# qcraftai/gedepth

Hardware: AMD Instinct MI355X
Metric: training img/s (whole node), KITTI-shaped 352x1120 synthetic batches (higher is better)
Workload: dtype bf16; 1 GPU; depthformer_swint_v: DepthFormer-SwinT + GEDepth-Vanilla, 352x1120, 8 img/GPU, full train step; global_batch=8, parallelism=dp1, allreduce_dtype=fp32, layout=nhwc, window_attention=bf16 mfma, params=53516992, hip_graph=off

## Files before the change

gedepth_amd/csrc/nhwc.hip:

```cpp
#include "common.h"

#define NH_MAXLANES 256

#define NH_MAXBLOCKS 1024
template <int K, int VN>
__device__ __forceinline__ void nh_col_commit(float (&acc)[K][VN], float* __restrict__ partial, int C, int lpr, int rpi, int c0) {
  __shared__ float sm[K][NH_MAXLANES][VN];
  const int t = threadIdx.x, rs = t / lpr;
#pragma unroll
  for (int k = 0; k < K; ++k)
#pragma unroll
    for (int v = 0; v < VN; ++v) sm[k][t][v] = acc[k][v];
  __syncthreads();
  int span = 1;
  while (span < rpi) span <<= 1;
  for (int stride = span >> 1; stride > 0; stride >>= 1) {
    if (rs < stride && rs + stride < rpi) {
#pragma unroll
      for (int k = 0; k < K; ++k)
#pragma unroll
        for (int v = 0; v < VN; ++v) sm[k][t][v] += sm[k][t + stride * lpr][v];
    }
    __syncthreads();
  }
  if (t < lpr) {
#pragma unroll
    for (int k = 0; k < K; ++k) {
      float* o = partial + ((long)blockIdx.x * K + k) * C + c0;
#pragma unroll
      for (int v = 0; v < VN; v += 4) *(float4*)(o + v) = make_float4(sm[k][t][v], sm[k][t][v + 1], sm[k][t][v + 2], sm[k][t][v + 3]);
    }
  }
}
template <typename O>
__global__ void __launch_bounds__(256) nh_partials_reduce_k(const float* __restrict__ partial, O* __restrict__ ws, int KC, int nb, int accumulate) {
  __shared__ double sm[8][32];
  const int j = threadIdx.x & 31, sl = threadIdx.x >> 5;
  const int kc = blockIdx.x * 32 + j;
  double a = 0.0;
  if (kc < KC) {
#pragma unroll 8
    for (int b = sl; b < nb; b += 8) a += (double)partial[(long)b * KC + kc];
  }
  sm[sl][j] = a;
  __syncthreads();
  if (sl == 0 && kc < KC) {
#pragma unroll
    for (int q = 1; q < 8; ++q) a += sm[q][j];
    ws[kc] = accumulate ? (O)((double)ws[kc] + a) : (O)a;
  }
}
static inline unsigned nh_grid_rows(long R, int rpi) { return ge_blocks(R, rpi * 8, NH_MAXBLOCKS); }
extern "C" size_t ge_nhwc_workspace(int C, int K) {
  return (size_t)C * ((size_t)K * sizeof(double) + 3 * sizeof(float) + (size_t)NH_MAXBLOCKS * K * sizeof(float));
}
static inline float* nh_partials(void* workspace, int C, int K) { return (float*)((char*)workspace + (size_t)C * (K * sizeof(double) + 3 * sizeof(float))); }
static inline void nh_reduce_launch_f32(void* workspace, int C, unsigned nb, float* out, int accumulate, hipStream_t s) {
  nh_partials_reduce_k<float><<<(C + 31) / 32, 256, 0, s>>>(nh_partials(workspace, C, 1), out, C, (int)nb, accumulate);
}
static inline void nh_reduce_launch(void* workspace, int C, int K, unsigned nb, hipStream_t s) {
  nh_partials_reduce_k<double><<<(K * C + 31) / 32, 256, 0, s>>>(nh_partials(workspace, C, K), (double*)workspace, K * C, (int)nb, 0);
}

template <typename T>
__global__ void __launch_bounds__(256) bn_stats_nhwc_k(const T* __restrict__ x, float* __restrict__ ws, int C, long R, int lpr, int rpi) {
  constexpr int VN = V8<T>::N;
  const int t = threadIdx.x, lane = t % lpr, rs = t / lpr;
  const int c0 = lane * VN;
  float acc[2][VN];
#pragma unroll
  for (int v = 0; v < VN; ++v) { acc[0][v] = 0.f; acc[1][v] = 0.f; }
  if (rs < rpi)
    for (long r = (long)blockIdx.x * rpi + rs; r < R; r += (long)gridDim.x * rpi) {
      float v[VN];
      V8<T>::ld(x + r * C + c0, v);
#pragma unroll
      for (int k = 0; k < VN; ++k) { acc[0][k] += v[k]; acc[1][k] += v[k] * v[k]; }
    }
  nh_col_commit<2, VN>(acc, ws, C, lpr, rpi, c0);
}
template <typename T>
__global__ void __launch_bounds__(256) bn_apply_nhwc_k(const T* __restrict__ x, const float* __restrict__ coef, T* __restrict__ y, int C,
                                                       long R, int lpr, int rpi, float slope) {
  constexpr int VN = V8<T>::N;
  const int t = threadIdx.x, lane = t % lpr, rs = t / lpr;
  if (rs >= rpi) return;
  const int c0 = lane * VN;
  float a[VN], b[VN];
#pragma unroll
  for (int k = 0; k < VN; ++k) { a[k] = coef[c0 + k]; b[k] = coef[C + c0 + k]; }
  for (long r = (long)blockIdx.x * rpi + rs; r < R; r += (long)gridDim.x * rpi) {
    float v[VN];
    V8<T>::ld(x + r * C + c0, v);
#pragma unroll
    for (int k = 0; k < VN; ++k) { const float tv = __fmaf_rn(v[k], a[k], b[k]); v[k] = tv > 0.f ? tv : tv * slope; }
    V8<T>::st(y + r * C + c0, v);
  }
}
template <typename T, bool RECOMP>
__global__ void __launch_bounds__(256) bn_bwd_stats_nhwc_k(const T* __restrict__ dy, const T* __restrict__ y, const T* __restrict__ x,
                                                           const float* __restrict__ gamma, const float* __restrict__ beta,
                                                           const float* __restrict__ save_mean, const float* __restrict__ save_rstd,
                                                           float* __restrict__ ws, int C, long R, int lpr, int rpi, float slope) {
  constexpr int VN = V8<T>::N;
  const int t = threadIdx.x, lane = t % lpr, rs = t / lpr;
  const int c0 = lane * VN;
  float mu[VN], rsd[VN], acc[2][VN], fa[VN], fb[VN];
#pragma unroll
  for (int v = 0; v < VN; ++v) {
    mu[v] = save_mean[c0 + v]; rsd[v] = save_rstd[c0 + v]; acc[0][v] = 0.f; acc[1][v] = 0.f;
    if (RECOMP) { fa[v] = gamma[c0 + v] * rsd[v]; fb[v] = __fmaf_rn(-mu[v], fa[v], beta[c0 + v]); }
  }
  if (rs < rpi)
    for (long r = (long)blockIdx.x * rpi + rs; r < R; r += (long)gridDim.x * rpi) {
      float g[VN], yv[VN], xv[VN];
      V8<T>::ld(dy + r * C + c0, g);
      V8<T>::ld(x + r * C + c0, xv);
      if (RECOMP) {
#pragma unroll
        for (int k = 0; k < VN; ++k) yv[k] = __fmaf_rn(xv[k], fa[k], fb[k]);
      } else {
        V8<T>::ld(y + r * C + c0, yv);
      }
#pragma unroll
      for (int k = 0; k < VN; ++k) {
        const float gg = yv[k] > 0.f ? g[k] : g[k] * slope;
        acc[0][k] += gg;
        acc[1][k] += gg * ((xv[k] - mu[k]) * rsd[k]);
      }
    }
  nh_col_commit<2, VN>(acc, ws, C, lpr, rpi, c0);
}
template <typename T, bool RECOMP>
__global__ void __launch_bounds__(256) bn_bwd_apply_nhwc_k(const T* __restrict__ dy, const T* __restrict__ y, const T* __restrict__ x,
                                                           const float* __restrict__ beta, const float* __restrict__ save_mean,
                                                           const float* __restrict__ save_rstd, const float* __restrict__ coef,
                                                           T* __restrict__ dx, int C, long R, int lpr, int rpi, float slope) {
  constexpr int VN = V8<T>::N;
  const int t = threadIdx.x, lane = t % lpr, rs = t / lpr;
  if (rs >= rpi) return;
  const int c0 = lane * VN;
  float a[VN], m1[VN], m2[VN], mu[VN], rsd[VN], fb[VN];
#pragma unroll
  for (int k = 0; k < VN; ++k) {
    a[k] = coef[c0 + k]; m1[k] = coef[C + c0 + k]; m2[k] = coef[2 * C + c0 + k]; mu[k] = save_mean[c0 + k]; rsd[k] = save_rstd[c0 + k];
    if (RECOMP) fb[k] = __fmaf_rn(-mu[k], a[k], beta[c0 + k]);
  }
  for (long r = (long)blockIdx.x * rpi + rs; r < R; r += (long)gridDim.x * rpi) {
    float g[VN], yv[VN], xv[VN];
    V8<T>::ld(dy + r * C + c0, g);
    V8<T>::ld(x + r * C + c0, xv);
    if (RECOMP) {
#pragma unroll
      for (int k = 0; k < VN; ++k) yv[k] = __fmaf_rn(xv[k], a[k], fb[k]);
    } else {
      V8<T>::ld(y + r * C + c0, yv);
    }
#pragma unroll
    for (int k = 0; k < VN; ++k) {
      const float gg = yv[k] > 0.f ? g[k] : g[k] * slope;
      g[k] = a[k] * (gg - m1[k] - ((xv[k] - mu[k]) * rsd[k]) * m2[k]);
    }
    V8<T>::st(dx + r * C + c0, g);
  }
}

__global__ void __launch_bounds__(256) bn_finalize_nhwc_k(const double* __restrict__ ws, const float* __restrict__ gamma,
                                                          const float* __restrict__ beta, float* __restrict__ save_mean,
                                                          float* __restrict__ save_rstd, float* __restrict__ running_mean,
                                                          float* __restrict__ running_var, float* __restrict__ coef, int C, double n,
                                                          float eps, float momentum) {
  const int c = blockIdx.x * blockDim.x + threadIdx.x;
  if (c >= C) return;
  const double mean = ws[c] / n;
  double var = ws[C + c] / n - mean * mean;
  if (var < 0.0) var = 0.0;
  const float rstd = (float)(1.0 / sqrt(var + (double)eps));
  save_mean[c] = (float)mean;
  save_rstd[c] = rstd;
  if (running_mean) running_mean[c] = (1.f - momentum) * running_mean[c] + momentum * (float)mean;
  if (running_var) running_var[c] = (1.f - momentum) * running_var[c] + momentum * (float)(n > 1.0 ? var * n / (n - 1.0) : var);
  const float a = gamma[c] * rstd;
  coef[c] = a;
  coef[C + c] = __fmaf_rn(-(float)mean, a, beta[c]);
}
__global__ void __launch_bounds__(256) bn_bwd_finalize_nhwc_k(const double* __restrict__ ws, const float* __restrict__ gamma,
                                                              const float* __restrict__ save_rstd, float* __restrict__ dgamma,
                                                              float* __restrict__ dbeta, float* __restrict__ coef, int C, double n) {
  const int c = blockIdx.x * blockDim.x + threadIdx.x;
  if (c >= C) return;
  dbeta[c] = (float)ws[c];
  dgamma[c] = (float)ws[C + c];
  coef[c] = gamma[c] * save_rstd[c];
  coef[C + c] = (float)(ws[c] / n);
  coef[2 * C + c] = (float)(ws[C + c] / n);
}

template <typename T> static bool nh_geom(int C, int& lpr, int& rpi) {
  constexpr int VN = V8<T>::N;
  if (C <= 0 || C % VN) return false;
  lpr = C / VN;
  if (lpr > NH_MAXLANES) return false;
  rpi = NH_MAXLANES / lpr;
  return true;
}
static inline bool nh_aligned(const void* a, const void* b = nullptr, const void* c = nullptr, const void* d = nullptr) {
  return ((((uintptr_t)a) | ((uintptr_t)b) | ((uintptr_t)c) | ((uintptr_t)d)) & 15) == 0;
}
static inline unsigned nh_grid_vec(long nvec) { return ge_blocks(nvec, 256 * 4, 65536); }
static inline unsigned nh_grid_apply(long R, int rpi) { return ge_blocks(R, rpi * 4, 16384); }

template <typename T>
static int bn_nhwc_fwd_launch(const void* x, const float* gamma, const float* beta, void* y, float* save_mean, float* save_rstd,
                              float* running_mean, float* running_var, void* workspace, long R, int C, float eps, float momentum,
                              float slope, hipStream_t s) {
  int lpr, rpi;
  if (!nh_geom<T>(C, lpr, rpi) || !nh_aligned(x, y)) return GE_ERR_UNSUPPORTED;
  double* ws = (double*)workspace;
  float* coef = (float*)(ws + 2 * C);
  const unsigned nb = nh_grid_rows(R, rpi);
  bn_stats_nhwc_k<T><<<nb, 256, 0, s>>>((const T*)x, nh_partials(workspace, C, 2), C, R, lpr, rpi);
  GE_LAUNCH_CHECK();
  nh_reduce_launch(workspace, C, 2, nb, s);
  GE_LAUNCH_CHECK();
  bn_finalize_nhwc_k<<<(C + 255) / 256, 256, 0, s>>>(ws, gamma, beta, save_mean, save_rstd, running_mean, running_var, coef, C, (double)R, eps, momentum);
  GE_LAUNCH_CHECK();
  bn_apply_nhwc_k<T><<<nh_grid_apply(R, rpi), 256, 0, s>>>((const T*)x, coef, (T*)y, C, R, lpr, rpi, slope);
  GE_LAUNCH_CHECK();
  return GE_OK;
}
template <typename T>
static int bn_nhwc_bwd_launch(const void* dy, const void* y, const void* x, const float* gamma, const float* beta, const float* save_mean,
                              const float* save_rstd, void* dx, float* dgamma, float* dbeta, void* workspace, long R, int C, float slope,
                              hipStream_t s) {
  int lpr, rpi;
  if (!nh_geom<T>(C, lpr, rpi) || !nh_aligned(dy, y, x, dx)) return GE_ERR_UNSUPPORTED;
  double* ws = (double*)workspace;
  float* coef = (float*)(ws + 2 * C);
  const unsigned nb = nh_grid_rows(R, rpi);
  float* part = nh_partials(workspace, C, 2);
  if (beta) bn_bwd_stats_nhwc_k<T, true><<<nb, 256, 0, s>>>((const T*)dy, nullptr, (const T*)x, gamma, beta, save_mean, save_rstd, part, C, R, lpr, rpi, slope);
  else bn_bwd_stats_nhwc_k<T, false><<<nb, 256, 0, s>>>((const T*)dy, (const T*)y, (const T*)x, gamma, beta, save_mean, save_rstd, part, C, R, lpr, rpi, slope);
  GE_LAUNCH_CHECK();
  nh_reduce_launch(workspace, C, 2, nb, s);
  GE_LAUNCH_CHECK();
  bn_bwd_finalize_nhwc_k<<<(C + 255) / 256, 256, 0, s>>>(ws, gamma, save_rstd, dgamma, dbeta, coef, C, (double)R);
  GE_LAUNCH_CHECK();
  if (beta) bn_bwd_apply_nhwc_k<T, true><<<nh_grid_apply(R, rpi), 256, 0, s>>>((const T*)dy, nullptr, (const T*)x, beta, save_mean, save_rstd, coef, (T*)dx, C, R, lpr, rpi, slope);
  else bn_bwd_apply_nhwc_k<T, false><<<nh_grid_apply(R, rpi), 256, 0, s>>>((const T*)dy, (const T*)y, (const T*)x, beta, save_mean, save_rstd, coef, (T*)dx, C, R, lpr, rpi, slope);
  GE_LAUNCH_CHECK();
  return GE_OK;
}
extern "C" int ge_bn_act_nhwc_fwd(const void* x, const float* gamma, const float* beta, void* y, float* save_mean, float* save_rstd,
                                  float* running_mean, float* running_var, void* workspace, long rows, int C, float eps,
                                  float momentum, float slope, int dtype, void* stream) {
  if (!x || !gamma || !beta || !y || !save_mean || !save_rstd || !workspace || rows <= 0 || C <= 0) return GE_ERR_BAD_ARG;
  if (dtype == GE_F32) return bn_nhwc_fwd_launch<float>(x, gamma, beta, y, save_mean, save_rstd, running_mean, running_var, workspace, rows, C, eps, momentum, slope, ge_stream(stream));
  if (dtype == GE_BF16) return bn_nhwc_fwd_launch<bf16_t>(x, gamma, beta, y, save_mean, save_rstd, running_mean, running_var, workspace, rows, C, eps, momentum, slope, ge_stream(stream));
  return GE_ERR_UNSUPPORTED;
}
extern "C" int ge_bn_act_nhwc_bwd(const void* dy, const void* y, const void* x, const float* gamma, const float* beta,
                                  const float* save_mean, const float* save_rstd, void* dx, float* dgamma, float* dbeta, void* workspace,
                                  long rows, int C, float slope, int dtype, void* stream) {
  if (!dy || (!y && !beta) || !x || !gamma || !save_mean || !save_rstd || !dx || !dgamma || !dbeta || !workspace || rows <= 0 || C <= 0) return GE_ERR_BAD_ARG;
  if (dtype == GE_F32) return bn_nhwc_bwd_launch<float>(dy, y, x, gamma, beta, save_mean, save_rstd, dx, dgamma, dbeta, workspace, rows, C, slope, ge_stream(stream));
  if (dtype == GE_BF16) return bn_nhwc_bwd_launch<bf16_t>(dy, y, x, gamma, beta, save_mean, save_rstd, dx, dgamma, dbeta, workspace, rows, C, slope, ge_stream(stream));
  return GE_ERR_UNSUPPORTED;
}

template <typename T>
__global__ void __launch_bounds__(256) bias_act_nhwc_fwd_k(T* __restrict__ x, const float* __restrict__ bias, int C, long R, int lpr, int rpi,
                                                           float slope) {
  constexpr int VN = V8<T>::N;
  const int t = threadIdx.x, lane = t % lpr, rs = t / lpr;
  if (rs >= rpi) return;
  const int c0 = lane * VN;
  float b[VN];
#pragma unroll
  for (int k = 0; k < VN; ++k) b[k] = bias[c0 + k];
  for (long r = (long)blockIdx.x * rpi + rs; r < R; r += (long)gridDim.x * rpi) {
    float v[VN];
    V8<T>::ld(x + r * C + c0, v);
#pragma unroll
    for (int k = 0; k < VN; ++k) { const float tv = v[k] + b[k]; v[k] = tv > 0.f ? tv : tv * slope; }
    V8<T>::st(x + r * C + c0, v);
  }
}
template <typename T>
__global__ void __launch_bounds__(256) bias_act_nhwc_bwd_k(const T* __restrict__ dy, const T* __restrict__ y, T* __restrict__ dx,
                                                           float* __restrict__ ws, int C, long R, int lpr, int rpi, float slope) {
  constexpr int VN = V8<T>::N;
  const int t = threadIdx.x, lane = t % lpr, rs = t / lpr;
  const int c0 = lane * VN;
  float acc[1][VN];
#pragma unroll
  for (int v = 0; v < VN; ++v) acc[0][v] = 0.f;
  if (rs < rpi)
    for (long r = (long)blockIdx.x * rpi + rs; r < R; r += (long)gridDim.x * rpi) {
      float g[VN], yv[VN];
      V8<T>::ld(dy + r * C + c0, g);
      V8<T>::ld(y + r * C + c0, yv);
#pragma unroll
      for (int k = 0; k < VN; ++k) { g[k] = yv[k] > 0.f ? g[k] : g[k] * slope; acc[0][k] += g[k]; }
      V8<T>::st(dx + r * C + c0, g);
    }
  nh_col_commit<1, VN>(acc, ws, C, lpr, rpi, c0);
}
extern "C" int ge_bias_act_nhwc_fwd(void* x, const float* bias, long rows, int C, float slope, int dtype, void* stream) {
  if (!x || !bias || rows <= 0 || C <= 0) return GE_ERR_BAD_ARG;
  int lpr, rpi;
  hipStream_t s = ge_stream(stream);
  if (dtype == GE_F32) {
    if (!nh_geom<float>(C, lpr, rpi) || !nh_aligned(x)) return GE_ERR_UNSUPPORTED;
    bias_act_nhwc_fwd_k<float><<<nh_grid_apply(rows, rpi), 256, 0, s>>>((float*)x, bias, C, rows, lpr, rpi, slope);
  } else if (dtype == GE_BF16) {
    if (!nh_geom<bf16_t>(C, lpr, rpi) || !nh_aligned(x)) return GE_ERR_UNSUPPORTED;
    bias_act_nhwc_fwd_k<bf16_t><<<nh_grid_apply(rows, rpi), 256, 0, s>>>((bf16_t*)x, bias, C, rows, lpr, rpi, slope);
  } else {
    return GE_ERR_UNSUPPORTED;
  }
  GE_LAUNCH_CHECK();
  return GE_OK;
}
extern "C" int ge_bias_act_nhwc_bwd(const void* dy, const void* y, void* dx, float* dbias, void* workspace, long rows, int C, float slope,
                                    int dtype, void* stream) {
  if (!dy || !y || !dx || !dbias || !workspace || rows <= 0 || C <= 0) return GE_ERR_BAD_ARG;
  int lpr, rpi;
  hipStream_t s = ge_stream(stream);
  double* ws = (double*)workspace;
  float* part = nh_partials(workspace, C, 1);
  unsigned nb = 1;
  if (dtype == GE_F32) {
    if (!nh_geom<float>(C, lpr, rpi) || !nh_aligned(dy, y, dx)) return GE_ERR_UNSUPPORTED;
    nb = nh_grid_rows(rows, rpi);
    bias_act_nhwc_bwd_k<float><<<nb, 256, 0, s>>>((const float*)dy, (const float*)y, (float*)dx, part, C, rows, lpr, rpi, slope);
  } else if (dtype == GE_BF16) {
    if (!nh_geom<bf16_t>(C, lpr, rpi) || !nh_aligned(dy, y, dx)) return GE_ERR_UNSUPPORTED;
    nb = nh_grid_rows(rows, rpi);
    bias_act_nhwc_bwd_k<bf16_t><<<nb, 256, 0, s>>>((const bf16_t*)dy, (const bf16_t*)y, (bf16_t*)dx, part, C, rows, lpr, rpi, slope);
  } else {
    return GE_ERR_UNSUPPORTED;
  }
  GE_LAUNCH_CHECK();
  nh_reduce_launch_f32(workspace, C, nb, dbias, 0, s);
  GE_LAUNCH_CHECK();
  return GE_OK;
}

template <typename T>
__global__ void __launch_bounds__(256) bilinear_nhwc_fwd_k(const T* __restrict__ in, T* __restrict__ out, int N, int Hi, int Wi, int Ho, int Wo,
                                                           int C, int lpr, int align) {
  constexpr int VN = V8<T>::N;
  const float sy = ge_scale(Hi, Ho, align), sx = ge_scale(Wi, Wo, align);
  const long total = (long)N * Ho * Wo * lpr;
  for (long idx = (long)blockIdx.x * 256 + threadIdx.x; idx < total; idx += (long)gridDim.x * 256) {
    const int c0 = (int)(idx % lpr) * VN;
    long t = idx / lpr;
    const int x = (int)(t % Wo); t /= Wo;
    const int y = (int)(t % Ho);
    const long n = t / Ho;
    const Lerp ly = ge_lerp(y, Hi, sy, align), lx = ge_lerp(x, Wi, sx, align);
    const T* base = in + n * (long)Hi * Wi * C + c0;
    float v00[VN], v01[VN], v10[VN], v11[VN], o[VN];
    V8<T>::ld(base + ((long)ly.i0 * Wi + lx.i0) * C, v00);
    V8<T>::ld(base + ((long)ly.i0 * Wi + lx.i1) * C, v01);
    V8<T>::ld(base + ((long)ly.i1 * Wi + lx.i0) * C, v10);
    V8<T>::ld(base + ((long)ly.i1 * Wi + lx.i1) * C, v11);
#pragma unroll
    for (int k = 0; k < VN; ++k) o[k] = ly.w0 * (lx.w0 * v00[k] + lx.w1 * v01[k]) + ly.w1 * (lx.w0 * v10[k] + lx.w1 * v11[k]);
    V8<T>::st(out + ((n * Ho + y) * (long)Wo + x) * C + c0, o);
  }
}
template <typename T>
__global__ void __launch_bounds__(256) bilinear_nhwc_bwd_k(const T* __restrict__ gout, T* __restrict__ gin, int N, int Hi, int Wi, int Ho, int Wo,
                                                           int C, int lpr, int align) {
  constexpr int VN = V8<T>::N;
  const float sy = ge_scale(Hi, Ho, align), sx = ge_scale(Wi, Wo, align);
  const long total = (long)N * Hi * Wi * lpr;
  for (long idx = (long)blockIdx.x * 256 + threadIdx.x; idx < total; idx += (long)gridDim.x * 256) {
    const int c0 = (int)(idx % lpr) * VN;
    long t = idx / lpr;
    const int X = (int)(t % Wi); t /= Wi;
    const int Y = (int)(t % Hi);
    const long n = t / Hi;
    int ylo, yhi, xlo, xhi;
    ge_cand_range<1>(Y, Ho, sy, align, ylo, yhi);
    ge_cand_range<1>(X, Wo, sx, align, xlo, xhi);
    const T* g = gout + n * (long)Ho * Wo * C + c0;
    float acc[VN];
#pragma unroll
    for (int k = 0; k < VN; ++k) acc[k] = 0.f;
    for (int oy = ylo; oy <= yhi; ++oy) {
      const Lerp ly = ge_lerp(oy, Hi, sy, align);
      const float wy = (ly.i0 == Y ? ly.w0 : 0.f) + (ly.i1 == Y ? ly.w1 : 0.f);
      if (wy == 0.f) continue;
      float row[VN];
#pragma unroll
      for (int k = 0; k < VN; ++k) row[k] = 0.f;
      for (int ox = xlo; ox <= xhi; ++ox) {
        const Lerp lx = ge_lerp(ox, Wi, sx, align);
        const float wx = (lx.i0 == X ? lx.w0 : 0.f) + (lx.i1 == X ? lx.w1 : 0.f);
        if (wx == 0.f) continue;
        float v[VN];
        V8<T>::ld(g + ((long)oy * Wo + ox) * C, v);
#pragma unroll
        for (int k = 0; k < VN; ++k) row[k] += wx * v[k];
      }
#pragma unroll
      for (int k = 0; k < VN; ++k) acc[k] += wy * row[k];
    }
    V8<T>::st(gin + ((n * Hi + Y) * (long)Wi + X) * C + c0, acc);
  }
}
template <typename T>
__global__ void __launch_bounds__(256) bilinear_nhwc_bwd_h_k(const T* __restrict__ gout, float* __restrict__ tmp, int N, int Wi, int Ho, int Wo,
                                                             int C, int lpr, int align) {
  constexpr int VN = V8<T>::N;
  const float sx = ge_scale(Wi, Wo, align);
  const long total = (long)N * Ho * Wi * lpr;
  for (long idx = (long)blockIdx.x * 256 + threadIdx.x; idx < total; idx += (long)gridDim.x * 256) {
    const int c0 = (int)(idx % lpr) * VN;
    long t = idx / lpr;
    const int X = (int)(t % Wi);
    const long row = t / Wi;
    int xlo, xhi;
    ge_cand_range<1>(X, Wo, sx, align, xlo, xhi);
    const T* g = gout + row * (long)Wo * C + c0;
    float acc[VN];
#pragma unroll
    for (int k = 0; k < VN; ++k) acc[k] = 0.f;
    for (int ox = xlo; ox <= xhi; ++ox) {
      const Lerp lx = ge_lerp(ox, Wi, sx, align);
      const float wx = (lx.i0 == X ? lx.w0 : 0.f) + (lx.i1 == X ? lx.w1 : 0.f);
      if (wx == 0.f) continue;
      float v[VN];
      V8<T>::ld(g + (long)ox * C, v);
#pragma unroll
      for (int k = 0; k < VN; ++k) acc[k] += wx * v[k];
    }
    float* o = tmp + (row * Wi + X) * (long)C + c0;
#pragma unroll
    for (int k = 0; k < VN; k += 4) *(float4*)(o + k) = make_float4(acc[k], acc[k + 1], acc[k + 2], acc[k + 3]);
  }
}
template <typename T>
__global__ void __launch_bounds__(256) bilinear_nhwc_bwd_v_k(const float* __restrict__ tmp, T* __restrict__ gin, int N, int Hi, int Wi, int Ho,
                                                             int C, int lpr, int align) {
  constexpr int VN = V8<T>::N;
  const float sy = ge_scale(Hi, Ho, align);
  const long total = (long)N * Hi * Wi * lpr;
  for (long idx = (long)blockIdx.x * 256 + threadIdx.x; idx < total; idx += (long)gridDim.x * 256) {
    const int c0 = (int)(idx % lpr) * VN;
    long t = idx / lpr;
    const int X = (int)(t % Wi); t /= Wi;
    const int Y = (int)(t % Hi);
    const long n = t / Hi;
    int ylo, yhi;
    ge_cand_range<1>(Y, Ho, sy, align, ylo, yhi);
    float acc[VN];
#pragma unroll
    for (int k = 0; k < VN; ++k) acc[k] = 0.f;
    for (int oy = ylo; oy <= yhi; ++oy) {
      const Lerp ly = ge_lerp(oy, Hi, sy, align);
      const float wy = (ly.i0 == Y ? ly.w0 : 0.f) + (ly.i1 == Y ? ly.w1 : 0.f);
      if (wy == 0.f) continue;
      const float* p = tmp + ((n * Ho + oy) * (long)Wi + X) * C + c0;
#pragma unroll
      for (int k = 0; k < VN; k += 4) {
        const float4 q = *(const float4*)(p + k);
        acc[k] += wy * q.x; acc[k + 1] += wy * q.y; acc[k + 2] += wy * q.z; acc[k + 3] += wy * q.w;
      }
    }
    V8<T>::st(gin + ((n * Hi + Y) * (long)Wi + X) * C + c0, acc);
  }
}

template <typename T>
static int bilinear_nhwc_launch(bool fwd, const void* src, void* dst, int N, int C, int Hi, int Wi, int Ho, int Wo, int align, hipStream_t s,
                                void* workspace = nullptr, size_t workspace_bytes = 0) {
  int lpr, rpi;
  if (!nh_geom<T>(C, lpr, rpi) || !nh_aligned(src, dst)) return GE_ERR_UNSUPPORTED;
  if (!fwd && workspace && (Ho > 3 * Hi || Wo > 3 * Wi) && workspace_bytes >= (size_t)N * Ho * Wi * C * sizeof(float) && nh_aligned(workspace)) {
    const long th = (long)N * Ho * Wi * lpr, tv = (long)N * Hi * Wi * lpr;
    if (th == 0 || tv == 0) return GE_OK;
    bilinear_nhwc_bwd_h_k<T><<<ge_blocks(th, 256, 1 << 18), 256, 0, s>>>((const T*)src, (float*)workspace, N, Wi, Ho, Wo, C, lpr, align);
    GE_LAUNCH_CHECK();
    bilinear_nhwc_bwd_v_k<T><<<ge_blocks(tv, 256, 1 << 18), 256, 0, s>>>((const float*)workspace, (T*)dst, N, Hi, Wi, Ho, C, lpr, align);
    GE_LAUNCH_CHECK();
    return GE_OK;
  }
  if (fwd) {
    const long total = (long)N * Ho * Wo * lpr;
    if (total == 0) return GE_OK;
    bilinear_nhwc_fwd_k<T><<<ge_blocks(total, 256, 1 << 18), 256, 0, s>>>((const T*)src, (T*)dst, N, Hi, Wi, Ho, Wo, C, lpr, align);
  } else {
    const long total = (long)N * Hi * Wi * lpr;
    if (total == 0) return GE_OK;
    bilinear_nhwc_bwd_k<T><<<ge_blocks(total, 256, 1 << 18), 256, 0, s>>>((const T*)src, (T*)dst, N, Hi, Wi, Ho, Wo, C, lpr, align);
  }
  GE_LAUNCH_CHECK();
  return GE_OK;
}
extern "C" int ge_bilinear_nhwc_fwd(const void* in, void* out, int N, int C, int Hi, int Wi, int Ho, int Wo, int align_corners, int dtype,
                                    void* stream) {
  if (!in || !out || N < 0 || C <= 0 || Hi <= 0 || Wi <= 0 || Ho <= 0 || Wo <= 0) return GE_ERR_BAD_ARG;
  if (dtype == GE_F32) return bilinear_nhwc_launch<float>(true, in, out, N, C, Hi, Wi, Ho, Wo, align_corners, ge_stream(stream));
  if (dtype == GE_BF16) return bilinear_nhwc_launch<bf16_t>(true, in, out, N, C, Hi, Wi, Ho, Wo, align_corners, ge_stream(stream));
  return GE_ERR_UNSUPPORTED;
}
extern "C" int ge_bilinear_nhwc_bwd(const void* d_out, void* d_in, void* workspace, size_t workspace_bytes, int N, int C, int Hi, int Wi, int Ho,
                                    int Wo, int align_corners, int dtype, void* stream) {
  if (!d_out || !d_in || N < 0 || C <= 0 || Hi <= 0 || Wi <= 0 || Ho <= 0 || Wo <= 0) return GE_ERR_BAD_ARG;
  if (dtype == GE_F32) return bilinear_nhwc_launch<float>(false, d_out, d_in, N, C, Hi, Wi, Ho, Wo, align_corners, ge_stream(stream), workspace, workspace_bytes);
  if (dtype == GE_BF16) return bilinear_nhwc_launch<bf16_t>(false, d_out, d_in, N, C, Hi, Wi, Ho, Wo, align_corners, ge_stream(stream), workspace, workspace_bytes);
  return GE_ERR_UNSUPPORTED;
}

template <typename T>
__global__ void __launch_bounds__(256) concat_rows_k(const T* __restrict__ a, long rpb, long a_bs, const T* __restrict__ res, const T* __restrict__ b,
                                                     T* __restrict__ out, long R, int Ca, int Cb, int off_a, int off_b, float p, float inv_keep,
                                                     uint64_t seed0, const unsigned long long* __restrict__ salt) {
  const uint64_t seed = ge_salted(seed0, salt);
  const uint32_t thr = ge_drop_threshold(p);
  constexpr int VN = V8<T>::N;
  const int la = Ca / VN, lb = b ? Cb / VN : 0, lt = la + lb, Co = Ca + Cb;
  const long total = R * lt;
  for (long i = (long)blockIdx.x * 256 + threadIdx.x; i < total; i += (long)gridDim.x * 256) {
    const long r = i / lt;
    const int j = (int)(i - r * lt);
    float v[VN];
    if (j < la) {
      const int c0 = j * VN;
      const long bi = r / rpb;
      V8<T>::ld(a + bi * a_bs + (r - bi * rpb) * Ca + c0, v);
      if (p > 0.f) {
#pragma unroll
        for (int k0 = 0; k0 < VN; k0 += 4) {
          float sc[4];
          ge_drop_scale4(seed, (uint64_t)(r * Ca + c0 + k0) >> 2, thr, inv_keep, sc);
#pragma unroll
          for (int e = 0; e < 4; ++e) v[k0 + e] *= sc[e];
        }
      }
      if (res) {
        float q[VN];
        V8<T>::ld(res + r * Ca + c0, q);
#pragma unroll
        for (int k = 0; k < VN; ++k) v[k] = Io<T>::rt(v[k]) + q[k];
      }
      V8<T>::st(out + r * Co + off_a + c0, v);
    } else {
      const int c0 = (j - la) * VN;
      V8<T>::ld(b + r * Cb + c0, v);
      V8<T>::st(out + r * Co + off_b + c0, v);
    }
  }
}
template <typename T>
__global__ void __launch_bounds__(256) slice_rows_drop_k(const T* __restrict__ d_out, T* __restrict__ d_a, long R, int Ca, int Co, int off_a,
                                                         float p, float inv_keep, uint64_t seed0, const unsigned long long* __restrict__ salt) {
  const uint64_t seed = ge_salted(seed0, salt);
  const uint32_t thr = ge_drop_threshold(p);
  constexpr int VN = V8<T>::N;
  const int la = Ca / VN;
  const long total = R * la;
  for (long i = (long)blockIdx.x * 256 + threadIdx.x; i < total; i += (long)gridDim.x * 256) {
    const long r = i / la;
    const int c0 = (int)(i - r * la) * VN;
    float v[VN];
    V8<T>::ld(d_out + r * Co + off_a + c0, v);
    if (p > 0.f) {
#pragma unroll
      for (int k0 = 0; k0 < VN; k0 += 4) {
        float sc[4];
        ge_drop_scale4(seed, (uint64_t)(r * Ca + c0 + k0) >> 2, thr, inv_keep, sc);
#pragma unroll
        for (int e = 0; e < 4; ++e) v[k0 + e] *= sc[e];
      }
    }
    V8<T>::st(d_a + r * Ca + c0, v);
  }
}
extern "C" int ge_concat_rows_fwd(const void* a, long rows_per_batch, long a_batch_stride, const void* res, const void* b, void* out, long rows,
                                  int Ca, int Cb, int a_first, float p_drop, unsigned long long seed, int dtype, void* stream) {
  if (!a || !out || rows <= 0 || Ca <= 0 || Cb < 0 || (Cb > 0 && !b) || p_drop < 0.f || p_drop >= 1.f) return GE_ERR_BAD_ARG;
  if (rows_per_batch <= 0 || rows % rows_per_batch || a_batch_stride < rows_per_batch * Ca) return GE_ERR_BAD_ARG;
  const int vn = dtype == GE_F32 ? 4 : 8;
  if ((dtype != GE_F32 && dtype != GE_BF16) || Ca % vn || Cb % vn || a_batch_stride % vn || !nh_aligned(a, res, b, out)) return GE_ERR_UNSUPPORTED;
  const int off_a = a_first ? 0 : Cb, off_b = a_first ? Ca : 0;
  const float inv_keep = p_drop > 0.f ? 1.f / (1.f - p_drop) : 1.f;
  const long total = rows * ((Ca + Cb) / vn);
  hipStream_t s = ge_stream(stream);
  if (dtype == GE_F32)
    concat_rows_k<float><<<nh_grid_vec(total), 256, 0, s>>>((const float*)a, rows_per_batch, a_batch_stride, (const float*)res, Cb ? (const float*)b : nullptr, (float*)out, rows, Ca, Cb, off_a, off_b, p_drop, inv_keep, seed, ge_rng_salt_get());
  else
    concat_rows_k<bf16_t><<<nh_grid_vec(total), 256, 0, s>>>((const bf16_t*)a, rows_per_batch, a_batch_stride, (const bf16_t*)res, Cb ? (const bf16_t*)b : nullptr, (bf16_t*)out, rows, Ca, Cb, off_a, off_b, p_drop, inv_keep, seed, ge_rng_salt_get());
  GE_LAUNCH_CHECK();
  return GE_OK;
}
extern "C" int ge_slice_rows_drop(const void* d_out, void* d_a, long rows, int Ca, int Co, int off_a, float p_drop, unsigned long long seed,
                                  int dtype, void* stream) {
  if (!d_out || !d_a || rows <= 0 || Ca <= 0 || Co < Ca || off_a < 0 || off_a + Ca > Co || p_drop < 0.f || p_drop >= 1.f) return GE_ERR_BAD_ARG;
  const int vn = dtype == GE_F32 ? 4 : 8;
  if ((dtype != GE_F32 && dtype != GE_BF16) || Ca % vn || Co % vn || off_a % vn || !nh_aligned(d_out, d_a)) return GE_ERR_UNSUPPORTED;
  const float inv_keep = p_drop > 0.f ? 1.f / (1.f - p_drop) : 1.f;
  hipStream_t s = ge_stream(stream);
  if (dtype == GE_F32)
    slice_rows_drop_k<float><<<nh_grid_vec(rows * (Ca / vn)), 256, 0, s>>>((const float*)d_out, (float*)d_a, rows, Ca, Co, off_a, p_drop, inv_keep, seed, ge_rng_salt_get());
  else
    slice_rows_drop_k<bf16_t><<<nh_grid_vec(rows * (Ca / vn)), 256, 0, s>>>((const bf16_t*)d_out, (bf16_t*)d_a, rows, Ca, Co, off_a, p_drop, inv_keep, seed, ge_rng_salt_get());
  GE_LAUNCH_CHECK();
  return GE_OK;
}

template <typename T>
__global__ void __launch_bounds__(256) add_rows_k(const T* __restrict__ x, const float* __restrict__ pos, T* __restrict__ out, long per_batch_vec,
                                                  long total_vec) {
  constexpr int VN = V8<T>::N;
  for (long i = (long)blockIdx.x * 256 + threadIdx.x; i < total_vec; i += (long)gridDim.x * 256) {
    const long j = i % per_batch_vec;
    float v[VN];
    V8<T>::ld(x + i * VN, v);
#pragma unroll
    for (int k = 0; k < VN; k += 4) {
      const float4 q = *(const float4*)(pos + j * VN + k);
      v[k] += q.x; v[k + 1] += q.y; v[k + 2] += q.z; v[k + 3] += q.w;
    }
    V8<T>::st(out + i * VN, v);
  }
}
extern "C" int ge_add_rows(const void* x, const float* pos, void* out, int B, long N, int C, int dtype, void* stream) {
  if (!x || !pos || !out || B <= 0 || N <= 0 || C <= 0) return GE_ERR_BAD_ARG;
  const int vn = dtype == GE_F32 ? 4 : 8;
  if ((dtype != GE_F32 && dtype != GE_BF16) || C % vn || !nh_aligned(x, pos, out)) return GE_ERR_UNSUPPORTED;
  const long per = N * C / vn, total = per * B;
  hipStream_t s = ge_stream(stream);
  if (dtype == GE_F32) add_rows_k<float><<<nh_grid_vec(total), 256, 0, s>>>((const float*)x, pos, (float*)out, per, total);
  else add_rows_k<bf16_t><<<nh_grid_vec(total), 256, 0, s>>>((const bf16_t*)x, pos, (bf16_t*)out, per, total);
  GE_LAUNCH_CHECK();
  return GE_OK;
}

template <typename T>
__global__ void __launch_bounds__(256) colsum_k(const T* __restrict__ x, float* __restrict__ ws, int C, long R, int lpr, int rpi) {
  constexpr int VN = V8<T>::N;
  const int t = threadIdx.x, lane = t % lpr, rs = t / lpr;
  const int c0 = (blockIdx.y * lpr + lane) * VN;
  float acc[1][VN];
#pragma unroll
  for (int v = 0; v < VN; ++v) acc[0][v] = 0.f;
  if (rs < rpi)
    for (long r = (long)blockIdx.x * rpi + rs; r < R; r += (long)gridDim.x * rpi) {
      float v[VN];
      V8<T>::ld(x + r * C + c0, v);
#pragma unroll
      for (int k = 0; k < VN; ++k) acc[0][k] += v[k];
    }
  nh_col_commit<1, VN>(acc, ws, C, lpr, rpi, c0);
}
template <typename T>
static int colsum_launch(const void* x, long R, int C, float* out, void* ws, int accumulate, hipStream_t s) {
  constexpr int VN = V8<T>::N;
  if (C % VN || !nh_aligned(x)) return GE_ERR_UNSUPPORTED;
  const int lanes = C / VN;
  int lpr = lanes < NH_MAXLANES ? lanes : NH_MAXLANES;
  while (lanes % lpr) --lpr;
  const int rpi = NH_MAXLANES / lpr, chunks = lanes / lpr;
  unsigned gx = nh_grid_rows(R, rpi);
  if (chunks > 1) gx = (gx + chunks - 1) / chunks;
  if (!gx) gx = 1;
  colsum_k<T><<<dim3(gx, chunks), 256, 0, s>>>((const T*)x, nh_partials(ws, C, 1), C, R, lpr, rpi);
  GE_LAUNCH_CHECK();
  nh_reduce_launch_f32(ws, C, gx, out, accumulate, s);
  GE_LAUNCH_CHECK();
  return GE_OK;
}
extern "C" int ge_colsum(const void* x, long R, int C, float* out, void* workspace, int accumulate, int dtype, void* stream) {
  if (!x || !out || !workspace || R < 0 || C <= 0) return GE_ERR_BAD_ARG;
  if (dtype == GE_F32) return colsum_launch<float>(x, R, C, out, workspace, accumulate, ge_stream(stream));
  if (dtype == GE_BF16) return colsum_launch<bf16_t>(x, R, C, out, workspace, accumulate, ge_stream(stream));
  return GE_ERR_UNSUPPORTED;
}

template <typename T> struct Gelu;
template <> struct Gelu<float> {
  static __device__ __forceinline__ float f(float x) { return 0.5f * x * (1.f + erff(x * 0.70710678118654752f)); }
  static __device__ __forceinline__ float grad(float x) {
    const float cdf = 0.5f * (1.f + erff(x * 0.70710678118654752f));
    return cdf + x * 0.3989422804014327f * expf(-0.5f * x * x);
  }
};
template <> struct Gelu<bf16_t> {
  static __device__ __forceinline__ void parts(float x, float& cdf, float& e) {
    const float z = fabsf(x) * 0.70710678118654752f;
    const float t = __builtin_amdgcn_rcpf(fmaf(0.3275911f, z, 1.f));
    e = __expf(-z * z);
    float p = fmaf(1.061405429f, t, -1.453152027f);
    p = fmaf(p, t, 1.421413741f); p = fmaf(p, t, -0.284496736f); p = fmaf(p, t, 0.254829592f);
    const float erfc_half = 0.5f * p * t * e;
    cdf = x >= 0.f ? 1.f - erfc_half : erfc_half;
  }
  static __device__ __forceinline__ float f(float x) { float c, e; parts(x, c, e); return x * c; }
  static __device__ __forceinline__ float grad(float x) { float c, e; parts(x, c, e); return fmaf(x * 0.3989422804014327f, e, c); }
};
template <typename T>
__global__ void __launch_bounds__(256) bias_gelu_fwd_k(const T* __restrict__ x, const float* __restrict__ bias, T* __restrict__ out, int C,
                                                       long R, int lpr, int rpi) {
  constexpr int VN = V8<T>::N;
  const int t = threadIdx.x, lane = t % lpr, rs = t / lpr;
  if (rs >= rpi) return;
  const int c0 = (blockIdx.y * lpr + lane) * VN;
  float b[VN];
#pragma unroll
  for (int k = 0; k < VN; ++k) b[k] = bias ? bias[c0 + k] : 0.f;
  for (long r = (long)blockIdx.x * rpi + rs; r < R; r += (long)gridDim.x * rpi) {
    float v[VN];
    V8<T>::ld(x + r * C + c0, v);
#pragma unroll
    for (int k = 0; k < VN; ++k) v[k] = Gelu<T>::f(v[k] + b[k]);
    V8<T>::st(out + r * C + c0, v);
  }
}
template <typename T>
__global__ void __launch_bounds__(256) bias_gelu_bwd_k(const T* __restrict__ dg, const T* __restrict__ x, const float* __restrict__ bias,
                                                       T* __restrict__ dy, float* __restrict__ ws, int C, long R, int lpr, int rpi) {
  constexpr int VN = V8<T>::N;
  const int t = threadIdx.x, lane = t % lpr, rs = t / lpr;
  const int c0 = (blockIdx.y * lpr + lane) * VN;
  float acc[1][VN], b[VN];
#pragma unroll
  for (int v = 0; v < VN; ++v) { acc[0][v] = 0.f; b[v] = bias ? bias[c0 + v] : 0.f; }
  if (rs < rpi)
    for (long r = (long)blockIdx.x * rpi + rs; r < R; r += (long)gridDim.x * rpi) {
      float g[VN], v[VN];
      V8<T>::ld(dg + r * C + c0, g);
      V8<T>::ld(x + r * C + c0, v);
#pragma unroll
      for (int k = 0; k < VN; ++k) {
        g[k] = Io<T>::rt(g[k] * Gelu<T>::grad(v[k] + b[k]));
        acc[0][k] += g[k];
      }
      V8<T>::st(dy + r * C + c0, g);
    }
  nh_col_commit<1, VN>(acc, ws, C, lpr, rpi, c0);
}
template <typename T>
static int bias_gelu_fwd_launch(const void* x, const float* bias, void* out, long R, int C, hipStream_t s) {
  constexpr int VN = V8<T>::N;
  if (C % VN || !nh_aligned(x, out)) return GE_ERR_UNSUPPORTED;
  const int lanes = C / VN;
  int lpr = lanes < NH_MAXLANES ? lanes : NH_MAXLANES;
  while (lanes % lpr) --lpr;
  const int rpi = NH_MAXLANES / lpr, chunks = lanes / lpr;
  bias_gelu_fwd_k<T><<<dim3(nh_grid_apply(R, rpi), chunks), 256, 0, s>>>((const T*)x, bias, (T*)out, C, R, lpr, rpi);
  GE_LAUNCH_CHECK();
  return GE_OK;
}
extern "C" int ge_bias_gelu_fwd(const void* x, const float* bias, void* out, long R, int C, int dtype, void* stream) {
  if (!x || !out || R < 0 || C <= 0) return GE_ERR_BAD_ARG;
  if (R == 0) return GE_OK;
  if (dtype == GE_F32) return bias_gelu_fwd_launch<float>(x, bias, out, R, C, ge_stream(stream));
  if (dtype == GE_BF16) return bias_gelu_fwd_launch<bf16_t>(x, bias, out, R, C, ge_stream(stream));
  return GE_ERR_UNSUPPORTED;
}
template <typename T>
static int bias_gelu_bwd_launch(const void* dg, const void* x, const float* bias, void* dy, float* d_bias, void* ws, long R, int C, hipStream_t s) {
  constexpr int VN = V8<T>::N;
  if (C % VN || !nh_aligned(dg, x, dy)) return GE_ERR_UNSUPPORTED;
  const int lanes = C / VN;
  int lpr = lanes < NH_MAXLANES ? lanes : NH_MAXLANES;
  while (lanes % lpr) --lpr;
  const int rpi = NH_MAXLANES / lpr, chunks = lanes / lpr;
  unsigned gx = nh_grid_rows(R, rpi);
  if (chunks > 1) gx = (gx + chunks - 1) / chunks;
  if (!gx) gx = 1;
  bias_gelu_bwd_k<T><<<dim3(gx, chunks), 256, 0, s>>>((const T*)dg, (const T*)x, bias, (T*)dy, nh_partials(ws, C, 1), C, R, lpr, rpi);
  GE_LAUNCH_CHECK();
  nh_reduce_launch_f32(ws, C, gx, d_bias, 0, s);
  GE_LAUNCH_CHECK();
  return GE_OK;
}
extern "C" int ge_bias_gelu_bwd(const void* dg, const void* x, const float* bias, void* dy, float* d_bias, void* workspace, long R, int C,
                                int dtype, void* stream) {
  if (!dg || !x || !dy || !d_bias || !workspace || R < 0 || C <= 0) return GE_ERR_BAD_ARG;
  if (dtype == GE_F32) return bias_gelu_bwd_launch<float>(dg, x, bias, dy, d_bias, workspace, R, C, ge_stream(stream));
  if (dtype == GE_BF16) return bias_gelu_bwd_launch<bf16_t>(dg, x, bias, dy, d_bias, workspace, R, C, ge_stream(stream));
  return GE_ERR_UNSUPPORTED;
}
```

gedepth_amd/depth/models/necks/hahi.py:

```python
import os

import torch
import torch.nn as nn
import torch.nn.functional as F

from .... import kernels as K
from ....kernels import add_rows, concat_tokens_map, ms_deform_attn_raw, residual_dropout, tokens_from_map
from ....mmrt import bricks
from ....mmrt.bricks import BaseModule, ConvModule, build_positional_encoding, xavier_init
from ..builder import ATTENTION, NECKS


@ATTENTION.register_module()
class MultiScaleDeformableAttention(BaseModule):

    def __init__(self, embed_dims=256, num_heads=8, num_levels=4, num_points=4, im2col_step=64, dropout=0.1,
                 batch_first=False, norm_cfg=None, init_cfg=None):
        super().__init__(init_cfg)
        if embed_dims % num_heads != 0:
            raise ValueError(f'embed_dims must be divisible by num_heads, but got {embed_dims} and {num_heads}')
        if embed_dims // num_heads != 64:
            raise NotImplementedError('the HIP sampling kernel is specialised for 64 channels per head')
        self.norm_cfg, self.batch_first = norm_cfg, batch_first
        self.dropout = nn.Dropout(dropout)
        self.im2col_step = im2col_step
        self.embed_dims, self.num_levels, self.num_heads, self.num_points = embed_dims, num_levels, num_heads, num_points
        self.sampling_offsets = nn.Linear(embed_dims, num_heads * num_levels * num_points * 2)
        self.attention_weights = nn.Linear(embed_dims, num_heads * num_levels * num_points)
        self.value_proj = bricks.Linear(embed_dims, embed_dims)
        self.output_proj = bricks.Linear(embed_dims, embed_dims)
        self.init_weights()

    def init_weights(self):
        bricks.constant_init(self.sampling_offsets, 0.)
        self.sampling_offsets.bias.data = bricks.msda_offset_bias(self.num_heads, self.num_levels, self.num_points)
        bricks.constant_init(self.attention_weights, val=0., bias=0.)
        xavier_init(self.value_proj, distribution='uniform', bias=0.)
        xavier_init(self.output_proj, distribution='uniform', bias=0.)
        self._is_init = True

    def _attend(self, query, value, reference_points, spatial_shapes, key_padding_mask=None, query_shapes=None, query_order=None):
        bs, num_query, _ = query.shape
        num_value = value.shape[1]
        if torch.is_tensor(spatial_shapes):
            spatial_shapes = [(int(h), int(w)) for h, w in spatial_shapes.tolist()]
        assert sum(h * w for h, w in spatial_shapes) == num_value
        if reference_points.shape[-1] != 2:
            raise ValueError('only 2-d reference points are used on the GEDepth path')
        value = self.value_proj(value)
        if key_padding_mask is not None:
            value = value.masked_fill(key_padding_mask[..., None], 0.0)
        value = value.view(bs, num_value, self.num_heads, -1)
        nH, L, P = self.num_heads, self.num_levels, self.num_points
        w = torch.cat((self.sampling_offsets.weight, self.attention_weights.weight), 0)
        b = torch.cat((self.sampling_offsets.bias, self.attention_weights.bias), 0)
        raw = bricks.linear_tokens(query, w, b)
        if raw.dtype != value.dtype:
            raw = raw.to(value.dtype)
        ref = reference_points.expand(bs, num_query, L, 2)
        if query_order is not None and 'msda_mm' not in K.DISABLED and K.msda_mm_supported(value, raw, spatial_shapes, nH, L, P):
            out = K.ms_deform_attn_mm(value, raw, ref, spatial_shapes, query_order, nH, L, P)
        elif K.msda_self_split_ok(value, raw, spatial_shapes, query_shapes, nH, L, P):
            out = K.ms_deform_attn_self_split(value, raw, ref, spatial_shapes, nH, L, P)
        else:
            out = ms_deform_attn_raw(value, raw, ref, spatial_shapes, query_shapes, nH, L, P)
        return self.output_proj(out)

    def forward(self, query, key=None, value=None, identity=None, query_pos=None, key_padding_mask=None,
                reference_points=None, spatial_shapes=None, level_start_index=None, query_shapes=None, query_order=None, **kwargs):
        if value is None:
            value = query
        if identity is None:
            identity = query
        if query_pos is not None:
            if query_pos.dim() == 3 and query_pos.shape[0] == 1 and query_pos.dtype == torch.float32 and query.dim() == 3 and self.batch_first:
                query = add_rows(query, query_pos[0])
            else:
                query = query + query_pos.to(query.dtype)
        if not self.batch_first:
            query, value = query.permute(1, 0, 2), value.permute(1, 0, 2)
        out = self._attend(query, value, reference_points, spatial_shapes, key_padding_mask, query_shapes, query_order)
        if not self.batch_first:
            out = out.permute(1, 0, 2)
        if self.training and self.dropout.p > 0 and out.is_cuda and out.dim() == 3 and self.batch_first:
            return residual_dropout(identity, out, self.dropout.p)
        return self.dropout(out) + identity

    def forward_map(self, fmap, pos_map, value, reference_points, spatial_shapes, concat_with, query_order=None, query=None):
        if query is None:
            query = tokens_from_map(fmap, pos_map)
        out = self._attend(query, value, reference_points, spatial_shapes, query_shapes=[tuple(fmap.shape[2:])], query_order=query_order)
        p = self.dropout.p if self.training else 0.0
        return concat_tokens_map(out, concat_with, identity=fmap, tokens_first=True, p_drop=p)


@NECKS.register_module()
class HAHIHeteroNeck(BaseModule):

    def __init__(self, in_channels, out_channels, embedding_dim, scales=[1, 1, 1, 1],
                 norm_cfg=dict(type='BN', requires_grad=True), act_cfg=dict(type='ReLU', inplace=True),
                 cross_att=True, self_att=True, constrain=False, positional_encoding=None, num_points=8):
        super().__init__()
        assert isinstance(in_channels, list)
        assert all(s == 1 for s in scales), 'GEDepth configs use scale 1 at every level'
        self.cross_att, self.self_att, self.constrain = cross_att, self_att, constrain
        self.in_channels, self.out_channels, self.scales = in_channels, out_channels, scales
        self.num_outs = len(scales)
        self.embedding_dim = E = embedding_dim
        cm = dict(norm_cfg=norm_cfg, act_cfg=act_cfg)
        self.lateral_convs = nn.ModuleList(ConvModule(i, o, kernel_size=1, **cm) for i, o in zip(in_channels, out_channels))
        self.trans_proj = nn.ModuleList(ConvModule(o, E, kernel_size=1, **cm) for o in out_channels[1:])
        self.trans_fusion = nn.ModuleList(ConvModule(o + E, o, kernel_size=3, padding=1, stride=1, **cm)
                                          for o in out_channels[1:])
        self.conv_proj = nn.Sequential(ConvModule(in_channels[0], E, kernel_size=1, **cm))
        self.conv_fusion = nn.Sequential(ConvModule(in_channels[0] + E, out_channels[0], kernel_size=3, padding=1,
                                                    stride=1, **cm))
        self.trans_positional_encoding = build_positional_encoding(positional_encoding)
        self.conv_positional_encoding = build_positional_encoding(positional_encoding)
        self.reference_points = nn.Linear(E, 2)
        self.level_embed = nn.Parameter(torch.Tensor(4, E))
        att = dict(embed_dims=E, num_levels=4, num_heads=8, num_points=num_points, batch_first=True)
        self.multi_att = MultiScaleDeformableAttention(**att)
        self.self_attn = MultiScaleDeformableAttention(**att)
        self._ref_cache = {}
        self._order_cache = {}

    ORDER_REFRESH = 64

    def _cross_order(self, ref_xy, level0_hw):
        key = (tuple(ref_xy.shape), tuple(level0_hw), str(ref_xy.device))
        ent = self._order_cache.get(key)
        stale = ent is not None and self.training and ent[1] >= self.ORDER_REFRESH and not torch.cuda.is_current_stream_capturing()
        if ent is None or stale:
            if len(self._order_cache) >= 8:
                self._order_cache.clear()
            ent = self._order_cache[key] = [K.msda_ref_order(ref_xy.detach(), level0_hw), 0]
        if self.training:
            ent[1] += 1
        return ent[0]

    def init_weights(self):
        for p in self.parameters():
            if p.dim() > 1:
                nn.init.xavier_uniform_(p)
        nn.init.xavier_uniform_(self.reference_points.weight.data, gain=1.0)
        nn.init.constant_(self.reference_points.bias.data, 0.)
        nn.init.normal_(self.level_embed)
        for m in self.modules():
            if isinstance(m, nn.Conv2d):
                xavier_init(m, distribution='uniform')
            if isinstance(m, MultiScaleDeformableAttention):
                m.init_weights()
        self._is_init = True

    def _pixel_centres(self, shapes, device):
        key = (tuple(shapes), str(device))
        if key not in self._ref_cache:
            pts = []
            for h, w in shapes:
                ry = torch.linspace(0.5, h - 0.5, h, dtype=torch.float32, device=device) / h
                rx = torch.linspace(0.5, w - 0.5, w, dtype=torch.float32, device=device) / w
                gy, gx = torch.meshgrid(ry, rx, indexing='ij')
                pts.append(torch.stack((gx.reshape(-1), gy.reshape(-1)), -1))
            ref = torch.cat(pts, 0)[None, :, None, :].expand(1, -1, len(shapes), 2).contiguous()
            self._ref_cache[key] = ref
        return self._ref_cache[key]

    def forward(self, inputs):
        assert len(inputs) == len(self.in_channels)
        feats = [conv(x) for conv, x in zip(self.lateral_convs, inputs)]
        feat_conv, feats_trans = feats[0], feats[1:]
        bs = feat_conv.shape[0]
        dev = feat_conv.device
        shapes, srcs, poss = [], [], []
        for i, ft in enumerate(feats_trans):
            h, w = ft.shape[2:]
            shapes.append((h, w))
            pos = self.trans_positional_encoding.grid(h, w, dev).flatten(2).transpose(1, 2)
            poss.append(pos + self.level_embed[i].view(1, 1, -1))
            srcs.append(self.trans_proj[i](ft).flatten(2).transpose(1, 2))
        src_flatten = torch.cat(srcs, 1)
        pos_flatten = torch.cat(poss, 1)
        if self.self_att:
            ref = self._pixel_centres(shapes, dev).expand(bs, -1, -1, -1)
            order = (K.msda_tile_order(shapes, dev) if (os.environ.get('GE_MSDA_MM_SELF') == '1' and src_flatten.is_cuda
                                                        and src_flatten.dtype == torch.bfloat16) else None)
            src = self.self_attn(src_flatten, value=None, identity=None, query_pos=pos_flatten,
                                 reference_points=ref, spatial_shapes=shapes, query_shapes=shapes, query_order=order)
        else:
            src = src_flatten

        h, w = feat_conv.shape[2:]
        pos_map = self.conv_positional_encoding.grid(h, w, dev) if self.cross_att else None
        query = None
        if self.training and len(self.conv_proj) == 1 and K.conv1x1_bn_act_pos_ok(self.conv_proj[0], feat_conv):
            conv_skip, query = K.conv1x1_bn_act_pos(self.conv_proj[0], feat_conv, pos_map)
        else:
            conv_skip = self.conv_proj(feat_conv)
        if self.cross_att:
            with torch.autocast('cuda', enabled=False):
                pm = pos_map.flatten(2)[0]
                w, b = self.reference_points.weight, self.reference_points.bias
                ref = torch.stack((torch.mv(pm.t(), w[0]), torch.mv(pm.t(), w[1])), -1).add(b).sigmoid()[None]
            order = self._cross_order(ref[0], shapes[0]) if (conv_skip.is_cuda and src.dtype == torch.bfloat16) else None
            ref = ref[:, :, None, :].expand(bs, -1, len(shapes), 2)
            fused = self.multi_att.forward_map(conv_skip, pos_map, src, ref, shapes, concat_with=feat_conv, query_order=order, query=query)
        else:
            fused = torch.cat([conv_skip, feat_conv], dim=1)
        outs = [self.conv_fusion(fused)]
        for i, (ft, piece) in enumerate(zip(feats_trans, torch.split(src, [h * w for h, w in shapes], dim=1))):
            outs.append(self.trans_fusion[i](concat_tokens_map(piece, ft, tokens_first=False)))
        return tuple(outs)
```

gedepth_amd/hip.py:

```python
import ctypes
import os
import re

import torch

_HERE = os.path.dirname(os.path.abspath(__file__))
LIB_PATH = os.environ.get('GE_LIB') or os.path.join(_HERE, 'csrc', 'libgedepth_hip.so')
HEADERS = {'SIGNATURES': 'gedepth_hip.h', 'EVAL_SIGNATURES': 'gedepth_eval.h', 'DDAD_SIGNATURES': 'gedepth_ddad.h',
           'CLOUD_SIGNATURES': 'gedepth_cloud.h', 'GROUND_SIGNATURES': 'gedepth_ground.h'}
EXTRA_HEADERS = {'BATCH_SIGNATURES': 'gedepth_batch.h'}
SCENE_HEADERS = {'SCENE_SIGNATURES': 'gedepth_scene.h'}
STRATA_HEADERS = {'STRATA_SIGNATURES': 'gedepth_strata.h'}
GE_F32, GE_BF16 = 0, 1
GE_COLORIZE_VMIN_DATA, GE_COLORIZE_VMAX_DATA, GE_COLORIZE_EQUAL = 1, 2, 4

_SCALARS = {'int': ctypes.c_int, 'long': ctypes.c_long, 'float': ctypes.c_float, 'double': ctypes.c_double, 'size_t': ctypes.c_size_t,
            'uint64_t': ctypes.c_ulonglong, 'unsigned long long': ctypes.c_ulonglong}
_DECL = re.compile(r'\b(int|size_t)\s+(ge_\w+)\s*\(([^()]*)\)\s*;')


def parse_header(text):
    text = re.sub(r'/\*.*?\*/|//[^\n]*', ' ', text, flags=re.S)
    sigs = {}
    for res, name, params in _DECL.findall(text):
        args = []
        for p in ([] if params.strip() == 'void' else params.split(',')):
            if '*' in p:
                args.append(ctypes.c_void_p)
                continue
            ctype = ' '.join(w for w in p.split()[:-1] if w != 'const')
            if ctype not in _SCALARS:
                raise TypeError(f'{name}: parameter "{" ".join(p.split())}" has a type the ctypes binding does not map')
            args.append(_SCALARS[ctype])
        sigs[name] = (_SCALARS[res], args)
    stray = set(re.findall(r'\b(ge_\w+)\s*\(', text)) - set(sigs)
    if stray:
        raise TypeError(f'cannot parse the declaration of {", ".join(sorted(stray))}')
    return sigs


for _table, _header in {**HEADERS, **EXTRA_HEADERS, **SCENE_HEADERS, **STRATA_HEADERS}.items():
    with open(os.path.join(os.path.dirname(_HERE), 'include', _header)) as _fh:
        globals()[_table] = parse_header(_fh.read())

_lib = None


class HipLibraryError(RuntimeError):
    pass


def lib():
    global _lib
    if _lib is None:
        if not os.path.isfile(LIB_PATH):
            raise HipLibraryError(
                f'{LIB_PATH} is missing: the gfx950 HIP kernels are not built. '
                f'Run gedepth_amd/csrc/build.sh (hipcc --offload-arch=gfx950). There is no CPU/eager fallback.')
        handle = ctypes.CDLL(LIB_PATH)
        for table in (*HEADERS, *EXTRA_HEADERS, *SCENE_HEADERS, *STRATA_HEADERS):
            for name, (res, args) in globals()[table].items():
                fn = getattr(handle, name)
                fn.restype, fn.argtypes = res, args
        _lib = handle
        if os.environ.get('GE_MSDA_MODE'):
            handle.ge_msda_mode(int(os.environ['GE_MSDA_MODE']))
    return _lib


def is_built():
    return os.path.isfile(LIB_PATH)


def check(code, what):
    if code != 0:
        raise RuntimeError(f'{what} failed with code {code} '
                           f'({"bad argument" if code == 10001 else "unsupported" if code == 10002 else "hipError_t"})')


def call(name, *args):
    code = getattr(_lib or lib(), name)(*args)
    if code:
        check(code, name)


def dtype_code(t):
    if t.dtype == torch.float32:
        return GE_F32
    if t.dtype == torch.bfloat16:
        return GE_BF16
    raise TypeError(f'gedepth_amd kernels take float32 or bfloat16 tensors, got {t.dtype}')


def ptr(t, dtype=None, name='tensor'):
    if t is None:
        return None
    if not t.is_cuda:
        raise RuntimeError(f'{name}: gedepth_amd ops run on MI355X only; got a {t.device} tensor '
                           '(the CPU oracle lives in oracle/ and is test infrastructure)')
    if not t.is_contiguous():
        raise RuntimeError(f'{name} must be contiguous')
    if dtype is not None and t.dtype != dtype:
        raise TypeError(f'{name} must be {dtype}, got {t.dtype}')
    return t.data_ptr()


def stream():
    return torch.cuda.current_stream().cuda_stream
```

gedepth_amd/mmrt/bricks.py:

```python
import math
import warnings

import torch
import torch.nn as nn
import torch.nn.functional as F

from .registry import Registry, build_from_cfg

MODELS = Registry('model')
ATTENTION = Registry('attention')
POSITIONAL_ENCODING = Registry('position encoding')
DROPOUT_LAYERS = Registry('drop out layers')


def constant_init(module, val, bias=0):
    if hasattr(module, 'weight') and module.weight is not None:
        nn.init.constant_(module.weight, val)
    if hasattr(module, 'bias') and module.bias is not None:
        nn.init.constant_(module.bias, bias)


def xavier_init(module, gain=1, bias=0, distribution='normal'):
    assert distribution in ['uniform', 'normal']
    if hasattr(module, 'weight') and module.weight is not None:
        if distribution == 'uniform':
            nn.init.xavier_uniform_(module.weight, gain=gain)
        else:
            nn.init.xavier_normal_(module.weight, gain=gain)
    if hasattr(module, 'bias') and module.bias is not None:
        nn.init.constant_(module.bias, bias)


def kaiming_init(module, a=0, mode='fan_out', nonlinearity='relu', bias=0, distribution='normal'):
    assert distribution in ['uniform', 'normal']
    if hasattr(module, 'weight') and module.weight is not None:
        if distribution == 'uniform':
            nn.init.kaiming_uniform_(module.weight, a=a, mode=mode, nonlinearity=nonlinearity)
        else:
            nn.init.kaiming_normal_(module.weight, a=a, mode=mode, nonlinearity=nonlinearity)
    if hasattr(module, 'bias') and module.bias is not None:
        nn.init.constant_(module.bias, bias)


def trunc_normal_init(module, mean=0., std=1., a=-2., b=2., bias=0.):
    if isinstance(module, torch.Tensor):
        nn.init.trunc_normal_(module, mean, std, a, b)
        return
    if hasattr(module, 'weight') and module.weight is not None:
        nn.init.trunc_normal_(module.weight, mean, std, a, b)
    if hasattr(module, 'bias') and module.bias is not None:
        nn.init.constant_(module.bias, bias)


class BaseModule(nn.Module):

    def __init__(self, init_cfg=None):
        super().__init__()
        self._is_init = False
        self.init_cfg = init_cfg

    @property
    def is_init(self):
        return self._is_init

    def init_weights(self):
        if self._is_init:
            warnings.warn(f'init_weights of {self.__class__.__name__} has been called more than once.')
            return
        for m in self.children():
            if hasattr(m, 'init_weights'):
                m.init_weights()
        self._is_init = True


class Sequential(BaseModule, nn.Sequential):

    def __init__(self, *args, init_cfg=None):
        BaseModule.__init__(self, init_cfg)
        nn.Sequential.__init__(self, *args)


class ModuleList(BaseModule, nn.ModuleList):

    def __init__(self, modules=None, init_cfg=None):
        BaseModule.__init__(self, init_cfg)
        nn.ModuleList.__init__(self, modules)


def _split_k(tokens):
    if tokens < 8192:
        return 0
    for s in range(64, 3, -1):
        if tokens % s == 0 and tokens // s >= 1024:
            return s
    return 0


def _linear_fwd(xc, wc, weight, bias, dt):
    from .. import kernels
    from .optim import lowp
    K = xc.shape[-1]
    M = xc.numel() // K
    if (dt == torch.bfloat16 and xc.is_cuda and xc.is_contiguous() and wc.is_contiguous() and kernels.gemm_own(M, K, wc.shape[0])
            and (bias is None or (bias.dtype == torch.float32 and bias.is_contiguous() and bias.data_ptr() % 16 == 0))
            and xc.data_ptr() % 16 == 0 and wc.data_ptr() % 16 == 0):
        return kernels.gemm_nt(xc.reshape(M, K), wc, None if bias is None else bias.detach()).view(*xc.shape[:-1], wc.shape[0])
    return F.linear(xc, wc, None if bias is None else lowp(bias, dt))


def _linear_dx(dy2, wc):
    from .. import kernels
    M, N = dy2.shape
    K = wc.shape[1]
    if dy2.dtype == torch.bfloat16 and dy2.is_contiguous() and dy2.data_ptr() % 16 == 0 and kernels.gemm_own(M, N, K):
        return kernels.gemm_nt(dy2, wc.t().contiguous(), None)
    return dy2 @ wc


def _sum_partials(part, weight, w_dtype):
    if weight is not None and w_dtype == torch.float32:
        from .optim import grad_target
        out = grad_target(weight)
        if out is not None and out.shape == part.shape[1:]:
            return torch.sum(part, 0, dtype=torch.float32, out=out)
    return part.sum(0, dtype=torch.float32).to(w_dtype)


def _plain_dw(dy2, x2, weight, w_dtype):
    if dy2.dtype == torch.bfloat16 and x2.dtype == torch.bfloat16 and w_dtype == torch.float32:
        from .. import kernels
        if 'mm_fp32_out' not in kernels.DISABLED:
            from .optim import grad_target
            out = grad_target(weight) if weight is not None else None
            if out is not None and tuple(out.shape) == (dy2.shape[1], x2.shape[1]):
                return torch.mm(dy2.t(), x2, out_dtype=torch.float32, out=out)
            return torch.mm(dy2.t(), x2, out_dtype=torch.float32)
    return _finished_grad(dy2.t() @ x2, weight, w_dtype)


def _finished_grad(dw, weight, w_dtype):
    from .optim import grad_into_arena
    return grad_into_arena(weight, dw, w_dtype) if weight is not None else dw.to(w_dtype)


class _LinearTokens(torch.autograd.Function):

    @staticmethod
    def forward(ctx, x, weight, bias, splits):
        dt = torch.get_autocast_dtype('cuda') if torch.is_autocast_enabled() else x.dtype
        with torch.autocast('cuda', enabled=False):
            from .optim import lowp
            xc, wc = x.to(dt), lowp(weight, dt)
            y = _linear_fwd(xc, wc, weight, bias, dt)
        ctx.save_for_backward(xc, wc)
        ctx.meta = (splits, x.dtype, weight.dtype, None if bias is None else bias.dtype)
        ctx.weight_ref = weight if isinstance(weight, nn.Parameter) else None
        return y

    @staticmethod
    def backward(ctx, dy):
        xc, wc = ctx.saved_tensors
        splits, x_dtype, w_dtype, b_dtype = ctx.meta
        K = xc.numel() // xc.shape[-1]
        with torch.autocast('cuda', enabled=False):
            dy2 = dy.to(wc.dtype).reshape(K, -1)
            x2 = xc.reshape(K, -1)
            dx = dw = db = None
            if not dy2.is_contiguous():
                dy2 = dy2.contiguous()
            if ctx.needs_input_grad[0]:
                dx = _linear_dx(dy2, wc).reshape(xc.shape).to(x_dtype)
            if ctx.needs_input_grad[1]:
                if splits:
                    M, N = dy2.shape[1], x2.shape[1]
                    part = torch.bmm(dy2.view(splits, K // splits, M).transpose(1, 2), x2.view(splits, K // splits, N))
                    dw = _sum_partials(part, ctx.weight_ref, w_dtype)
                else:
                    dw = _plain_dw(dy2, x2, ctx.weight_ref, w_dtype)
            if b_dtype is not None and ctx.needs_input_grad[2]:
                if dy2.shape[1] % (4 if dy2.dtype == torch.float32 else 8) == 0:
                    from .. import kernels
                    db = kernels.colsum(dy2 if dy2.is_contiguous() else dy2.contiguous()).to(b_dtype)
                else:
                    db = dy2.sum(0, dtype=torch.float32).to(b_dtype)
        return dx, dw, db, None


class _LinearBiasGelu(torch.autograd.Function):

    @staticmethod
    def forward(ctx, x, weight, bias, splits):
        from .. import kernels
        dt = torch.get_autocast_dtype('cuda') if torch.is_autocast_enabled() else x.dtype
        with torch.autocast('cuda', enabled=False):
            from .optim import lowp
            xc, wc = x.to(dt), lowp(weight, dt)
            y0 = _linear_fwd(xc, wc, weight, bias, dt)
            g = kernels.bias_gelu_fwd(y0, None)
        ctx.save_for_backward(xc, wc, y0)
        ctx.meta = (splits, x.dtype, weight.dtype, bias.dtype)
        ctx.weight_ref = weight if isinstance(weight, nn.Parameter) else None
        return g

    @staticmethod
    def backward(ctx, dg):
        from .. import kernels
        xc, wc, y0 = ctx.saved_tensors
        splits, x_dtype, w_dtype, b_dtype = ctx.meta
        K = xc.numel() // xc.shape[-1]
        with torch.autocast('cuda', enabled=False):
            dg2 = dg.to(wc.dtype).reshape(K, -1)
            if not dg2.is_contiguous():
                dg2 = dg2.contiguous()
            dy2, db = kernels.bias_gelu_bwd(dg2, y0.reshape(K, -1), None)
            x2 = xc.reshape(K, -1)
            dx = dw = None
            if ctx.needs_input_grad[0]:
                dx = _linear_dx(dy2, wc).reshape(xc.shape).to(x_dtype)
            if ctx.needs_input_grad[1]:
                if splits:
                    M, N = dy2.shape[1], x2.shape[1]
                    part = torch.bmm(dy2.view(splits, K // splits, M).transpose(1, 2), x2.view(splits, K // splits, N))
                    dw = _sum_partials(part, ctx.weight_ref, w_dtype)
                else:
                    dw = _plain_dw(dy2, x2, ctx.weight_ref, w_dtype)
        return dx, dw, (db.to(b_dtype) if ctx.needs_input_grad[2] else None), None


def linear_bias_gelu(x, weight, bias):
    C = weight.shape[0]
    ok = (x.is_cuda and torch.is_grad_enabled() and weight.requires_grad and bias is not None and x.dim() >= 2 and x.numel() > 0
          and x.dtype in (torch.float32, torch.bfloat16) and C % 8 == 0)
    if ok:
        from .. import kernels
        ok = 'bias_gelu' not in kernels.DISABLED
    if not ok:
        return F.gelu(linear_tokens(x, weight, bias))
    return _LinearBiasGelu.apply(x, weight, bias, _split_k(x.numel() // x.shape[-1]))


def linear_tokens(x, weight, bias=None):
    if not (x.is_cuda and torch.is_grad_enabled() and weight.requires_grad) or x.dtype not in (torch.float32, torch.bfloat16) or x.dim() < 2 or x.numel() == 0:
        return F.linear(x, weight, bias)
    return _LinearTokens.apply(x, weight, bias, _split_k(x.numel() // x.shape[-1]))


class Linear(nn.Linear):

    def forward(self, x):
        return linear_tokens(x, self.weight, self.bias)


class LayerNorm(nn.LayerNorm):
    autocast_out = True

    def _hip_ok(self, x):
        C = x.shape[-1]
        return (x.is_cuda and self.elementwise_affine and len(self.normalized_shape) == 1 and C % 4 == 0 and C <= 3072
                and x.dtype in (torch.float32, torch.bfloat16))

    def _out_dtype(self, x):
        if torch.is_autocast_enabled():
            return torch.get_autocast_dtype('cuda') if self.autocast_out else torch.float32
        return x.dtype

    def forward_with_skip(self, x):
        if self._hip_ok(x) and torch.is_grad_enabled() and x.requires_grad:
            from .. import kernels
            if 'ln_res' not in kernels.DISABLED:
                return kernels.layer_norm_res(x, self.weight, self.bias, self.eps, self._out_dtype(x))
        return self(x), x

    def forward(self, x):
        C = x.shape[-1]
        if self._hip_ok(x):
            from .. import kernels
            return kernels.layer_norm(x, self.weight, self.bias, self.eps, self._out_dtype(x))
        if x.is_cuda:
            from .. import kernels
            kernels.note_fallback('LayerNorm', f'C={C} dtype={x.dtype}')
        return super().forward(x)


_NORM = {
    'BN': ('bn', nn.BatchNorm2d), 'BN1d': ('bn', nn.BatchNorm1d), 'BN2d': ('bn', nn.BatchNorm2d),
    'SyncBN': ('bn', nn.SyncBatchNorm), 'GN': ('gn', nn.GroupNorm), 'LN': ('ln', LayerNorm),
    'IN': ('in', nn.InstanceNorm2d),
}
_ACT = {
    'ReLU': nn.ReLU, 'LeakyReLU': nn.LeakyReLU, 'PReLU': nn.PReLU, 'ReLU6': nn.ReLU6, 'ELU': nn.ELU,
    'Sigmoid': nn.Sigmoid, 'Tanh': nn.Tanh, 'GELU': nn.GELU,
}
_CONV = {'Conv1d': nn.Conv1d, 'Conv2d': nn.Conv2d, 'Conv3d': nn.Conv3d, 'Conv': nn.Conv2d}


def build_norm_layer(cfg, num_features, postfix=''):
    if not isinstance(cfg, dict) or 'type' not in cfg:
        raise KeyError('the cfg dict must contain the key "type"')
    cfg_ = dict(cfg)
    layer_type = cfg_.pop('type')
    if layer_type not in _NORM:
        raise KeyError(f'Unrecognized norm type {layer_type}')
    abbr, norm_layer = _NORM[layer_type]
    name = abbr + str(postfix)
    requires_grad = cfg_.pop('requires_grad', True)
    cfg_.setdefault('eps', 1e-5)
    if layer_type == 'GN':
        assert 'num_groups' in cfg_
        layer = norm_layer(num_channels=num_features, **cfg_)
    else:
        layer = norm_layer(num_features, **cfg_)
    for p in layer.parameters():
        p.requires_grad = requires_grad
    return name, layer


def build_activation_layer(cfg):
    cfg_ = dict(cfg)
    t = cfg_.pop('type')
    if t not in _ACT:
        raise KeyError(f'Unrecognized activation type {t}')
    return _ACT[t](**cfg_)


def build_conv_layer(cfg, *args, **kwargs):
    cfg_ = dict(type='Conv2d') if cfg is None else dict(cfg)
    t = cfg_.pop('type')
    if t not in _CONV:
        raise KeyError(f'Unrecognized conv type {t}')
    return _CONV[t](*args, **kwargs, **cfg_)


class ConvModule(nn.Module):

    def __init__(self, in_channels, out_channels, kernel_size, stride=1, padding=0, dilation=1, groups=1,
                 bias='auto', conv_cfg=None, norm_cfg=None, act_cfg=dict(type='ReLU'), inplace=True,
                 order=('conv', 'norm', 'act')):
        super().__init__()
        assert order == ('conv', 'norm', 'act'), 'only the conv-norm-act order is on the GEDepth path'
        self.conv_cfg, self.norm_cfg, self.act_cfg = conv_cfg, norm_cfg, act_cfg
        self.inplace = inplace
        self.with_norm = norm_cfg is not None
        self.with_activation = act_cfg is not None
        if bias == 'auto':
            bias = not self.with_norm
        self.with_bias = bias
        self.conv = build_conv_layer(conv_cfg, in_channels, out_channels, kernel_size, stride=stride,
                                     padding=padding, dilation=dilation, groups=groups, bias=bias)
        self.in_channels, self.out_channels = in_channels, out_channels
        if self.with_norm:
            self.norm_name, norm = build_norm_layer(norm_cfg, out_channels)
            self.add_module(self.norm_name, norm)
        else:
            self.norm_name = None
        if self.with_activation:
            act_cfg_ = dict(act_cfg)
            if act_cfg_['type'] not in ['Tanh', 'PReLU', 'Sigmoid', 'GELU']:
                act_cfg_.setdefault('inplace', inplace)
            self.activate = build_activation_layer(act_cfg_)
        self.init_weights()

    @property
    def norm(self):
        return getattr(self, self.norm_name) if self.norm_name else None

    def init_weights(self):
        if self.with_activation and self.act_cfg['type'] == 'LeakyReLU':
            nonlinearity, a = 'leaky_relu', self.act_cfg.get('negative_slope', 0.01)
        else:
            nonlinearity, a = 'relu', 0
        kaiming_init(self.conv, a=a, nonlinearity=nonlinearity)
        if self.with_norm:
            constant_init(self.norm, 1, bias=0)

    def _fused_slope(self):
        if self.with_norm or self.conv.bias is None or type(self.conv) is not nn.Conv2d:
            return None
        if not self.with_activation:
            return 1.0
        if isinstance(self.activate, nn.LeakyReLU):
            return float(self.activate.negative_slope)
        if isinstance(self.activate, nn.ReLU):
            return 0.0
        return None

    def _fused_bn_slope(self):
        bn = self.norm
        if (type(bn) is not nn.BatchNorm2d or not bn.training or not bn.affine or not bn.track_running_stats
                or bn.momentum is None or self.conv.bias is not None):
            return None
        if not self.with_activation:
            return 1.0
        if isinstance(self.activate, nn.ReLU):
            return 0.0
        if isinstance(self.activate, nn.LeakyReLU):
            return float(self.activate.negative_slope)
        return None

    def forward(self, x):
        slope = self._fused_slope() if x.is_cuda else None
        if slope is not None:
            return conv_bias_act(self.conv, x, slope)
        if x.is_cuda and self.conv.bias is None:
            from .. import kernels
            if kernels.conv3x3_ok(self.conv, x):
                x = kernels.conv3x3(self.conv, x)
            else:
                x = kernels.conv_lib(self.conv, x)
        else:
            x = self.conv(x)
        if x.is_cuda and self.with_norm and x.dtype in (torch.float32, torch.bfloat16):
            slope = self._fused_bn_slope()
            if slope is not None:
                from .. import kernels
                return kernels.bn_act(x, self.norm, slope)
        if x.is_cuda and (self.with_norm or self.with_activation) and self.training:
            from .. import kernels
            kernels.note_fallback('ConvModule', f'norm={type(self.norm).__name__ if self.with_norm else None} act={self.act_cfg}')
        if self.with_norm:
            x = self.norm(x)
        if self.with_activation:
            x = self.activate(x)
        return x


def conv_bias_act(conv, x, slope=1.0):
    from .. import kernels
    if kernels.conv3x3_ok(conv, x):
        return kernels.conv3x3(conv, x, conv.bias, act=slope != 1.0, slope=slope)
    if slope == 1.0 and kernels.conv3x3_c1_ok(conv, x):
        return kernels.conv3x3_c1(conv, x)
    y = kernels.conv_lib(conv, x)
    if not (y.is_contiguous() or kernels._cl_ok(y)):
        y = y.contiguous()
    return kernels.bias_act_(y, conv.bias, slope)


def drop_path(x, drop_prob=0., training=False):
    if drop_prob == 0. or not training:
        return x
    keep_prob = 1 - drop_prob
    shape = (x.shape[0],) + (1,) * (x.ndim - 1)
    random_tensor = keep_prob + torch.rand(shape, dtype=x.dtype, device=x.device)
    return x.div(keep_prob) * random_tensor.floor()


@DROPOUT_LAYERS.register_module()
class DropPath(nn.Module):

    def __init__(self, drop_prob=0.1):
        super().__init__()
        self.drop_prob = drop_prob

    def forward(self, x):
        return drop_path(x, self.drop_prob, self.training)

    def residual(self, identity, branch):
        if (not identity.is_cuda or self.drop_prob == 0. or not self.training or identity.shape != branch.shape
                or (identity.dtype, branch.dtype) not in _RESIDUAL_DTYPES):
            if identity.is_cuda and self.training and self.drop_prob > 0.:
                from .. import kernels
                kernels.note_fallback('DropPath.residual', f'{identity.dtype}+{branch.dtype} {tuple(identity.shape)} vs {tuple(branch.shape)}')
            return identity + self(branch)
        from .. import kernels
        return kernels.residual_drop_path(identity, branch, _DROP_PATH_BANK.scale(self, branch.shape[0], branch.dtype, branch.device))


class _DropPathBank:

    def __init__(self):
        self.layers, self.rows, self.used, self.key, self.keep = [], None, [], None, None
        self.probs = None
        self.seed, self.offset = None, 0

    def scale(self, layer, batch, dtype, device):
        idx = getattr(layer, '_bank_index', None)
        key = (batch, device)
        if idx is None or idx >= len(self.layers) or self.layers[idx]() is not layer:
            import weakref
            self.layers = [r for r in self.layers if r() is not None]
            for i, r in enumerate(self.layers):
                r()._bank_index = i
            idx = layer._bank_index = len(self.layers)
            self.layers.append(weakref.ref(layer))
            self.rows = self.keep = None
        gen = torch.cuda.default_generators[device.index if device.index is not None else torch.cuda.current_device()] if device.type == 'cuda' else None
        capturing = gen is not None and torch.cuda.is_current_stream_capturing()
        reseeded = gen is not None and not capturing and (gen.initial_seed(), gen.get_offset() >= self.offset) != (self.seed, True)
        if self.rows is None or self.key != key or self.used[idx] or reseeded:
            probs = [1.0 - (r().drop_prob if r() is not None else 0.0) for r in self.layers]
            if self.keep is None or self.keep.device != device or probs != self.probs:
                self.keep, self.probs = torch.tensor(probs, dtype=torch.float32).view(-1, 1).to(device), probs
            u = torch.rand((len(self.layers), batch), dtype=torch.float32, device=device)
            self.rows = (self.keep + u).floor() / self.keep
            self.used = [False] * len(self.layers)
            self.key = key
            if gen is not None and not capturing:
                self.seed, self.offset = gen.initial_seed(), gen.get_offset()
        self.used[idx] = True
        return self.rows[idx]


_DROP_PATH_BANK = _DropPathBank()


_RESIDUAL_DTYPES = {(torch.float32, torch.float32), (torch.float32, torch.bfloat16), (torch.bfloat16, torch.bfloat16)}


@DROPOUT_LAYERS.register_module()
class Dropout(nn.Dropout):

    def __init__(self, drop_prob=0.5, inplace=False):
        super().__init__(p=drop_prob, inplace=inplace)


def build_dropout(cfg, default_args=None):
    return build_from_cfg(cfg, DROPOUT_LAYERS, default_args)


def build_positional_encoding(cfg, default_args=None):
    return build_from_cfg(cfg, POSITIONAL_ENCODING, default_args)


class FFN(BaseModule):

    def __init__(self, embed_dims=256, feedforward_channels=1024, num_fcs=2,
                 act_cfg=dict(type='ReLU', inplace=True), ffn_drop=0., dropout_layer=None,
                 add_identity=True, init_cfg=None, **kwargs):
        super().__init__(init_cfg)
        assert num_fcs >= 2
        self.embed_dims, self.feedforward_channels, self.num_fcs = embed_dims, feedforward_channels, num_fcs
        self.act_cfg = act_cfg
        self.activate = build_activation_layer(act_cfg)
        layers, in_channels = [], embed_dims
        for _ in range(num_fcs - 1):
            layers.append(Sequential(Linear(in_channels, feedforward_channels), self.activate,
                                     nn.Dropout(ffn_drop)))
            in_channels = feedforward_channels
        layers.append(Linear(feedforward_channels, embed_dims))
        layers.append(nn.Dropout(ffn_drop))
        self.layers = Sequential(*layers)
        self.dropout_layer = build_dropout(dropout_layer) if dropout_layer else nn.Identity()
        self.add_identity = add_identity

    def _fused_first(self):
        first = self.layers[0]
        return (self.num_fcs == 2 and isinstance(first, nn.Sequential) and len(first) == 3 and type(first[0]) is Linear
                and type(first[1]) is nn.GELU and getattr(first[1], 'approximate', 'none') == 'none'
                and isinstance(first[2], nn.Dropout) and (first[2].p == 0 or not self.training))

    def forward(self, x, identity=None):
        if x.is_cuda and self._fused_first():
            lin = self.layers[0][0]
            h = linear_bias_gelu(x, lin.weight, lin.bias)
            out = self.layers[2](self.layers[1](h))
        else:
            out = self.layers(x)
        if not self.add_identity:
            return self.dropout_layer(out)
        if identity is None:
            identity = x
        if hasattr(self.dropout_layer, 'residual'):
            return self.dropout_layer.residual(identity, out)
        return identity + self.dropout_layer(out)


def msda_offset_bias(num_heads, num_levels, num_points):
    thetas = torch.arange(num_heads, dtype=torch.float32) * (2.0 * math.pi / num_heads)
    grid = torch.stack([thetas.cos(), thetas.sin()], -1)
    grid = (grid / grid.abs().max(-1, keepdim=True)[0]).view(num_heads, 1, 1, 2).repeat(
        1, num_levels, num_points, 1)
    for i in range(num_points):
        grid[:, :, i, :] *= i + 1
    return grid.view(-1)
```

Measured before the change: 171.4 img/s.

## Fuse neck level BN-act writes into concatenated token buffer with strided row kernels

Adds row-strided variants of the NHWC BN+activation forward and backward kernels, so each pyramid level's output is written straight into, and its gradient read straight from, a shared multi-level token buffer. This avoids separate flatten and concat copies. It also adds kernels that apply per-level positional and level embeddings in one pass, compute the embedding gradient as per-level column sums, and sum fan-out token gradients from strided parts. The goal is fewer elementwise launches and less memory traffic in the DepthFormer neck, at the cost of more index arithmetic per row and more custom autograd code.

```diff
diff --git a/gedepth_amd/csrc/nhwc.hip b/gedepth_amd/csrc/nhwc.hip
--- a/gedepth_amd/csrc/nhwc.hip
+++ b/gedepth_amd/csrc/nhwc.hip
@@ -1,4 +1,5 @@
 #include "common.h"
+#include "../../include/gedepth_neck.h"
 
 #define NH_MAXLANES 256
 
@@ -62,6 +63,21 @@
   nh_partials_reduce_k<double><<<(K * C + 31) / 32, 256, 0, s>>>(nh_partials(workspace, C, K), (double*)workspace, K * C, (int)nb, 0);
 }
 
+struct NhWalk {
+  int img, n, nl, sb, sn;
+  __device__ __forceinline__ NhWalk(unsigned r0, unsigned step, int nl_) : nl(nl_) {
+    const unsigned d = (unsigned)nl_;
+    img = (int)(r0 / d); n = (int)(r0 - (unsigned)img * d);
+    sb = (int)(step / d); sn = (int)(step - (unsigned)sb * d);
+  }
+  __device__ __forceinline__ void next() {
+    n += sn; img += sb;
+    if (n >= nl) { n -= nl; ++img; }
+  }
+  __device__ __forceinline__ long row(long image_stride) const { return (long)img * image_stride + n; }
+};
+#define NH_WALK_MAX_ROWS (1 << 30)
+
 template <typename T>
 __global__ void __launch_bounds__(256) bn_stats_nhwc_k(const T* __restrict__ x, float* __restrict__ ws, int C, long R, int lpr, int rpi) {
   constexpr int VN = V8<T>::N;
@@ -79,9 +95,9 @@
     }
   nh_col_commit<2, VN>(acc, ws, C, lpr, rpi, c0);
 }
-template <typename T>
+template <typename T, bool ROWS = false>
 __global__ void __launch_bounds__(256) bn_apply_nhwc_k(const T* __restrict__ x, const float* __restrict__ coef, T* __restrict__ y, int C,
-                                                       long R, int lpr, int rpi, float slope) {
+                                                       long R, int lpr, int rpi, float slope, int npi = 0, long istr = 0) {
   constexpr int VN = V8<T>::N;
   const int t = threadIdx.x, lane = t % lpr, rs = t / lpr;
   if (rs >= rpi) return;
@@ -89,19 +105,22 @@
   float a[VN], b[VN];
 #pragma unroll
   for (int k = 0; k < VN; ++k) { a[k] = coef[c0 + k]; b[k] = coef[C + c0 + k]; }
+  NhWalk w(blockIdx.x * rpi + rs, gridDim.x * rpi, ROWS ? npi : 1);
   for (long r = (long)blockIdx.x * rpi + rs; r < R; r += (long)gridDim.x * rpi) {
     float v[VN];
     V8<T>::ld(x + r * C + c0, v);
 #pragma unroll
     for (int k = 0; k < VN; ++k) { const float tv = __fmaf_rn(v[k], a[k], b[k]); v[k] = tv > 0.f ? tv : tv * slope; }
-    V8<T>::st(y + r * C + c0, v);
-  }
-}
-template <typename T, bool RECOMP>
+    if (ROWS) { V8<T>::st(y + w.row(istr) * C + c0, v); w.next(); }
+    else V8<T>::st(y + r * C + c0, v);
+  }
+}
+template <typename T, bool RECOMP, bool ROWS = false>
 __global__ void __launch_bounds__(256) bn_bwd_stats_nhwc_k(const T* __restrict__ dy, const T* __restrict__ y, const T* __restrict__ x,
                                                            const float* __restrict__ gamma, const float* __restrict__ beta,
                                                            const float* __restrict__ save_mean, const float* __restrict__ save_rstd,
-                                                           float* __restrict__ ws, int C, long R, int lpr, int rpi, float slope) {
+                                                           float* __restrict__ ws, int C, long R, int lpr, int rpi, float slope, int npi = 0,
+                                                           long istr = 0) {
   constexpr int VN = V8<T>::N;
   const int t = threadIdx.x, lane = t % lpr, rs = t / lpr;
   const int c0 = lane * VN;
@@ -111,10 +130,12 @@
     mu[v] = save_mean[c0 + v]; rsd[v] = save_rstd[c0 + v]; acc[0][v] = 0.f; acc[1][v] = 0.f;
     if (RECOMP) { fa[v] = gamma[c0 + v] * rsd[v]; fb[v] = __fmaf_rn(-mu[v], fa[v], beta[c0 + v]); }
   }
+  NhWalk w(blockIdx.x * rpi + rs, gridDim.x * rpi, ROWS ? npi : 1);
   if (rs < rpi)
     for (long r = (long)blockIdx.x * rpi + rs; r < R; r += (long)gridDim.x * rpi) {
       float g[VN], yv[VN], xv[VN];
-      V8<T>::ld(dy + r * C + c0, g);
+      if (ROWS) { V8<T>::ld(dy + w.row(istr) * C + c0, g); w.next(); }
+      else V8<T>::ld(dy + r * C + c0, g);
       V8<T>::ld(x + r * C + c0, xv);
       if (RECOMP) {
 #pragma unroll
@@ -131,11 +152,12 @@
     }
   nh_col_commit<2, VN>(acc, ws, C, lpr, rpi, c0);
 }
-template <typename T, bool RECOMP>
+template <typename T, bool RECOMP, bool ROWS = false>
 __global__ void __launch_bounds__(256) bn_bwd_apply_nhwc_k(const T* __restrict__ dy, const T* __restrict__ y, const T* __restrict__ x,
                                                            const float* __restrict__ beta, const float* __restrict__ save_mean,
                                                            const float* __restrict__ save_rstd, const float* __restrict__ coef,
-                                                           T* __restrict__ dx, int C, long R, int lpr, int rpi, float slope) {
+                                                           T* __restrict__ dx, int C, long R, int lpr, int rpi, float slope, int npi = 0,
+                                                           long istr = 0) {
   constexpr int VN = V8<T>::N;
   const int t = threadIdx.x, lane = t % lpr, rs = t / lpr;
   if (rs >= rpi) return;
@@ -146,9 +168,11 @@
     a[k] = coef[c0 + k]; m1[k] = coef[C + c0 + k]; m2[k] = coef[2 * C + c0 + k]; mu[k] = save_mean[c0 + k]; rsd[k] = save_rstd[c0 + k];
     if (RECOMP) fb[k] = __fmaf_rn(-mu[k], a[k], beta[c0 + k]);
   }
+  NhWalk w(blockIdx.x * rpi + rs, gridDim.x * rpi, ROWS ? npi : 1);
   for (long r = (long)blockIdx.x * rpi + rs; r < R; r += (long)gridDim.x * rpi) {
     float g[VN], yv[VN], xv[VN];
-    V8<T>::ld(dy + r * C + c0, g);
+    if (ROWS) { V8<T>::ld(dy + w.row(istr) * C + c0, g); w.next(); }
+    else V8<T>::ld(dy + r * C + c0, g);
     V8<T>::ld(x + r * C + c0, xv);
     if (RECOMP) {
 #pragma unroll
@@ -213,7 +237,7 @@
 template <typename T>
 static int bn_nhwc_fwd_launch(const void* x, const float* gamma, const float* beta, void* y, float* save_mean, float* save_rstd,
                               float* running_mean, float* running_var, void* workspace, long R, int C, float eps, float momentum,
-                              float slope, hipStream_t s) {
+                              float slope, hipStream_t s, long npi = 0, long istr = 0) {
   int lpr, rpi;
   if (!nh_geom<T>(C, lpr, rpi) || !nh_aligned(x, y)) return GE_ERR_UNSUPPORTED;
   double* ws = (double*)workspace;
@@ -225,28 +249,31 @@
   GE_LAUNCH_CHECK();
   bn_finalize_nhwc_k<<<(C + 255) / 256, 256, 0, s>>>(ws, gamma, beta, save_mean, save_rstd, running_mean, running_var, coef, C, (double)R, eps, momentum);
   GE_LAUNCH_CHECK();
-  bn_apply_nhwc_k<T><<<nh_grid_apply(R, rpi), 256, 0, s>>>((const T*)x, coef, (T*)y, C, R, lpr, rpi, slope);
+  if (npi) bn_apply_nhwc_k<T, true><<<nh_grid_apply(R, rpi), 256, 0, s>>>((const T*)x, coef, (T*)y, C, R, lpr, rpi, slope, (int)npi, istr);
+  else bn_apply_nhwc_k<T><<<nh_grid_apply(R, rpi), 256, 0, s>>>((const T*)x, coef, (T*)y, C, R, lpr, rpi, slope);
   GE_LAUNCH_CHECK();
   return GE_OK;
 }
 template <typename T>
 static int bn_nhwc_bwd_launch(const void* dy, const void* y, const void* x, const float* gamma, const float* beta, const float* save_mean,
                               const float* save_rstd, void* dx, float* dgamma, float* dbeta, void* workspace, long R, int C, float slope,
-                              hipStream_t s) {
+                              hipStream_t s, long npi = 0, long istr = 0) {
   int lpr, rpi;
   if (!nh_geom<T>(C, lpr, rpi) || !nh_aligned(dy, y, x, dx)) return GE_ERR_UNSUPPORTED;
   double* ws = (double*)workspace;
   float* coef = (float*)(ws + 2 * C);
   const unsigned nb = nh_grid_rows(R, rpi);
   float* part = nh_partials(workspace, C, 2);
-  if (beta) bn_bwd_stats_nhwc_k<T, true><<<nb, 256, 0, s>>>((const T*)dy, nullptr, (const T*)x, gamma, beta, save_mean, save_rstd, part, C, R, lpr, rpi, slope);
+  if (npi) bn_bwd_stats_nhwc_k<T, true, true><<<nb, 256, 0, s>>>((const T*)dy, nullptr, (const T*)x, gamma, beta, save_mean, save_rstd, part, C, R, lpr, rpi, slope, (int)npi, istr);
+  else if (beta) bn_bwd_stats_nhwc_k<T, true><<<nb, 256, 0, s>>>((const T*)dy, nullptr, (const T*)x, gamma, beta, save_mean, save_rstd, part, C, R, lpr, rpi, slope);
   else bn_bwd_stats_nhwc_k<T, false><<<nb, 256, 0, s>>>((const T*)dy, (const T*)y, (const T*)x, gamma, beta, save_mean, save_rstd, part, C, R, lpr, rpi, slope);
   GE_LAUNCH_CHECK();
   nh_reduce_launch(workspace, C, 2, nb, s);
   GE_LAUNCH_CHECK();
   bn_bwd_finalize_nhwc_k<<<(C + 255) / 256, 256, 0, s>>>(ws, gamma, save_rstd, dgamma, dbeta, coef, C, (double)R);
   GE_LAUNCH_CHECK();
-  if (beta) bn_bwd_apply_nhwc_k<T, true><<<nh_grid_apply(R, rpi), 256, 0, s>>>((const T*)dy, nullptr, (const T*)x, beta, save_mean, save_rstd, coef, (T*)dx, C, R, lpr, rpi, slope);
+  if (npi) bn_bwd_apply_nhwc_k<T, true, true><<<nh_grid_apply(R, rpi), 256, 0, s>>>((const T*)dy, nullptr, (const T*)x, beta, save_mean, save_rstd, coef, (T*)dx, C, R, lpr, rpi, slope, (int)npi, istr);
+  else if (beta) bn_bwd_apply_nhwc_k<T, true><<<nh_grid_apply(R, rpi), 256, 0, s>>>((const T*)dy, nullptr, (const T*)x, beta, save_mean, save_rstd, coef, (T*)dx, C, R, lpr, rpi, slope);
   else bn_bwd_apply_nhwc_k<T, false><<<nh_grid_apply(R, rpi), 256, 0, s>>>((const T*)dy, (const T*)y, (const T*)x, beta, save_mean, save_rstd, coef, (T*)dx, C, R, lpr, rpi, slope);
   GE_LAUNCH_CHECK();
   return GE_OK;
@@ -265,6 +292,25 @@
   if (!dy || (!y && !beta) || !x || !gamma || !save_mean || !save_rstd || !dx || !dgamma || !dbeta || !workspace || rows <= 0 || C <= 0) return GE_ERR_BAD_ARG;
   if (dtype == GE_F32) return bn_nhwc_bwd_launch<float>(dy, y, x, gamma, beta, save_mean, save_rstd, dx, dgamma, dbeta, workspace, rows, C, slope, ge_stream(stream));
   if (dtype == GE_BF16) return bn_nhwc_bwd_launch<bf16_t>(dy, y, x, gamma, beta, save_mean, save_rstd, dx, dgamma, dbeta, workspace, rows, C, slope, ge_stream(stream));
+  return GE_ERR_UNSUPPORTED;
+}
+static inline bool nh_rows_ok(long rows, long npi, long istr) { return npi > 0 && npi <= NH_WALK_MAX_ROWS && rows % npi == 0 && istr >= npi; }
+extern "C" int ge_bn_act_nhwc_fwd_rows(const void* x, const float* gamma, const float* beta, void* y, long rows_per_image, long image_stride,
+                                       float* save_mean, float* save_rstd, float* running_mean, float* running_var, void* workspace, long rows,
+                                       int C, float eps, float momentum, float slope, int dtype, void* stream) {
+  if (!x || !gamma || !beta || !y || !save_mean || !save_rstd || !workspace || rows <= 0 || C <= 0) return GE_ERR_BAD_ARG;
+  if (!nh_rows_ok(rows, rows_per_image, image_stride)) return GE_ERR_BAD_ARG;
+  if (dtype == GE_F32) return bn_nhwc_fwd_launch<float>(x, gamma, beta, y, save_mean, save_rstd, running_mean, running_var, workspace, rows, C, eps, momentum, slope, ge_stream(stream), rows_per_image, image_stride);
+  if (dtype == GE_BF16) return bn_nhwc_fwd_launch<bf16_t>(x, gamma, beta, y, save_mean, save_rstd, running_mean, running_var, workspace, rows, C, eps, momentum, slope, ge_stream(stream), rows_per_image, image_stride);
+  return GE_ERR_UNSUPPORTED;
+}
+extern "C" int ge_bn_act_nhwc_bwd_rows(const void* dy, long rows_per_image, long image_stride, const void* x, const float* gamma,
+                                       const float* beta, const float* save_mean, const float* save_rstd, void* dx, float* dgamma, float* dbeta,
+                                       void* workspace, long rows, int C, float slope, int dtype, void* stream) {
+  if (!dy || !beta || !x || !gamma || !save_mean || !save_rstd || !dx || !dgamma || !dbeta || !workspace || rows <= 0 || C <= 0) return GE_ERR_BAD_ARG;
+  if (!nh_rows_ok(rows, rows_per_image, image_stride)) return GE_ERR_BAD_ARG;
+  if (dtype == GE_F32) return bn_nhwc_bwd_launch<float>(dy, nullptr, x, gamma, beta, save_mean, save_rstd, dx, dgamma, dbeta, workspace, rows, C, slope, ge_stream(stream), rows_per_image, image_stride);
+  if (dtype == GE_BF16) return bn_nhwc_bwd_launch<bf16_t>(dy, nullptr, x, gamma, beta, save_mean, save_rstd, dx, dgamma, dbeta, workspace, rows, C, slope, ge_stream(stream), rows_per_image, image_stride);
   return GE_ERR_UNSUPPORTED;
 }
 
@@ -682,6 +728,170 @@
   return GE_ERR_UNSUPPORTED;
 }
 
+struct NhLevels { int s[GE_NECK_MAX_LEVELS + 1]; };
+struct NhParts { const void* p[GE_NECK_MAX_LEVELS]; long pitch[GE_NECK_MAX_LEVELS]; long col[GE_NECK_MAX_LEVELS]; };
+static bool nh_levels(const long* starts, int n, long N, NhLevels& lv, long& longest) {
+  if (!starts || n < 1 || n > GE_NECK_MAX_LEVELS || N <= 0 || N > NH_WALK_MAX_ROWS || starts[0] != 0 || starts[n] != N) return false;
+  longest = 0;
+  for (int l = 0; l <= GE_NECK_MAX_LEVELS; ++l) lv.s[l] = (int)N;
+  for (int l = 0; l < n; ++l) {
+    if (starts[l + 1] < starts[l]) return false;
+    lv.s[l] = (int)starts[l];
+    if (starts[l + 1] - starts[l] > longest) longest = starts[l + 1] - starts[l];
+  }
+  return true;
+}
+
+template <typename T>
+__global__ void __launch_bounds__(256) add_rows_levels_k(const T* __restrict__ x, const float* __restrict__ pos, const float* __restrict__ emb,
+                                                         T* __restrict__ out, int B, long N, int C, NhLevels lv, int lpr, int rpi) {
+  constexpr int VN = V8<T>::N;
+  const int t = threadIdx.x, lane = t % lpr, rs = t / lpr, level = blockIdx.y;
+  const int start = lv.s[level], nl = lv.s[level + 1] - start;
+  if (rs >= rpi || nl <= 0) return;
+  const int c0 = lane * VN;
+  float e[VN];
+#pragma unroll
+  for (int k = 0; k < VN; ++k) e[k] = emb[(long)level * C + c0 + k];
+  const long R = (long)B * nl;
+  NhWalk w(blockIdx.x * rpi + rs, gridDim.x * rpi, nl);
+  for (long r = (long)blockIdx.x * rpi + rs; r < R; r += (long)gridDim.x * rpi, w.next()) {
+    const long o = (w.row(N) + start) * C + c0;
+    const float* q = pos + (long)(start + w.n) * C + c0;
+    float v[VN];
+    V8<T>::ld(x + o, v);
+#pragma unroll
+    for (int k = 0; k < VN; k += 4) {
+      const float4 p4 = *(const float4*)(q + k);
+      v[k] += p4.x + e[k]; v[k + 1] += p4.y + e[k + 1]; v[k + 2] += p4.z + e[k + 2]; v[k + 3] += p4.w + e[k + 3];
+    }
+    V8<T>::st(out + o, v);
+  }
+}
+extern "C" int ge_add_rows_levels(const void* x, const float* pos, const float* emb, void* out, int B, long N, int C, const long* level_starts,
+                                  int n_levels, int dtype, void* stream) {
+  NhLevels lv;
+  long longest;
+  if (!x || !pos || !emb || !out || B <= 0 || C <= 0 || !nh_levels(level_starts, n_levels, N, lv, longest)) return GE_ERR_BAD_ARG;
+  int lpr, rpi;
+  if (dtype != GE_F32 && dtype != GE_BF16) return GE_ERR_UNSUPPORTED;
+  if (!(dtype == GE_F32 ? nh_geom<float>(C, lpr, rpi) : nh_geom<bf16_t>(C, lpr, rpi)) || !nh_aligned(x, pos, out)) return GE_ERR_UNSUPPORTED;
+  const dim3 grid(nh_grid_apply((long)B * longest, rpi), n_levels);
+  hipStream_t s = ge_stream(stream);
+  if (dtype == GE_F32) add_rows_levels_k<float><<<grid, 256, 0, s>>>((const float*)x, pos, emb, (float*)out, B, N, C, lv, lpr, rpi);
+  else add_rows_levels_k<bf16_t><<<grid, 256, 0, s>>>((const bf16_t*)x, pos, emb, (bf16_t*)out, B, N, C, lv, lpr, rpi);
+  GE_LAUNCH_CHECK();
+  return GE_OK;
+}
+
+template <typename T>
+__global__ void __launch_bounds__(256) level_colsum_k(const T* __restrict__ x, float* __restrict__ ws, int B, long N, int C, int L, NhLevels lv,
+                                                      int lpr, int rpi) {
+  constexpr int VN = V8<T>::N;
+  const int t = threadIdx.x, lane = t % lpr, rs = t / lpr, level = blockIdx.y;
+  const int start = lv.s[level], nl = lv.s[level + 1] - start;
+  const int c0 = lane * VN;
+  float acc[1][VN];
+#pragma unroll
+  for (int v = 0; v < VN; ++v) acc[0][v] = 0.f;
+  if (rs < rpi && nl > 0) {
+    const long R = (long)B * nl;
+    NhWalk w(blockIdx.x * rpi + rs, gridDim.x * rpi, nl);
+    for (long r = (long)blockIdx.x * rpi + rs; r < R; r += (long)gridDim.x * rpi, w.next()) {
+      float v[VN];
+      V8<T>::ld(x + (w.row(N) + start) * C + c0, v);
+#pragma unroll
+      for (int k = 0; k < VN; ++k) acc[0][k] += v[k];
+    }
+  }
+  nh_col_commit<1, VN>(acc, ws + (long)level * C, L * C, lpr, rpi, c0);
+}
+extern "C" int ge_level_colsum(const void* x, int B, long N, int C, const long* level_starts, int n_levels, float* out, void* workspace,
+                               int dtype, void* stream) {
+  NhLevels lv;
+  long longest;
+  if (!x || !out || !workspace || B <= 0 || C <= 0 || !nh_levels(level_starts, n_levels, N, lv, longest)) return GE_ERR_BAD_ARG;
+  int lpr, rpi;
+  if (dtype != GE_F32 && dtype != GE_BF16) return GE_ERR_UNSUPPORTED;
+  if (!(dtype == GE_F32 ? nh_geom<float>(C, lpr, rpi) : nh_geom<bf16_t>(C, lpr, rpi)) || !nh_aligned(x, out)) return GE_ERR_UNSUPPORTED;
+  const unsigned gx = nh_grid_rows((long)B * longest, rpi);
+  float* part = nh_partials(workspace, C, n_levels);
+  hipStream_t s = ge_stream(stream);
+  if (dtype == GE_F32) level_colsum_k<float><<<dim3(gx, n_levels), 256, 0, s>>>((const float*)x, part, B, N, C, n_levels, lv, lpr, rpi);
+  else level_colsum_k<bf16_t><<<dim3(gx, n_levels), 256, 0, s>>>((const bf16_t*)x, part, B, N, C, n_levels, lv, lpr, rpi);
+  GE_LAUNCH_CHECK();
+  nh_partials_reduce_k<float><<<(n_levels * C + 31) / 32, 256, 0, s>>>(part, out, n_levels * C, (int)gx, 0);
+  GE_LAUNCH_CHECK();
+  return GE_OK;
+}
+
+template <typename T>
+__global__ void __launch_bounds__(256) token_grad_sum_k(const T* __restrict__ a0, const T* __restrict__ a1, const T* __restrict__ a2,
+                                                        NhParts pt, int has_parts, T* __restrict__ out, int B, long N, int C, NhLevels lv,
+                                                        int lpr, int rpi) {
+  constexpr int VN = V8<T>::N;
+  const int t = threadIdx.x, lane = t % lpr, rs = t / lpr, level = blockIdx.y;
+  const int start = lv.s[level], nl = lv.s[level + 1] - start;
+  if (rs >= rpi || nl <= 0) return;
+  const int c0 = lane * VN;
+  const T* part = has_parts ? (const T*)pt.p[level] + pt.col[level] + c0 : nullptr;
+  const long pitch = has_parts ? pt.pitch[level] : 0;
+  const long R = (long)B * nl;
+  NhWalk w(blockIdx.x * rpi + rs, gridDim.x * rpi, nl);
+  for (long r = (long)blockIdx.x * rpi + rs; r < R; r += (long)gridDim.x * rpi, w.next()) {
+    const long o = (w.row(N) + start) * C + c0;
+    float v[VN], q[VN];
+#pragma unroll
+    for (int k = 0; k < VN; ++k) v[k] = 0.f;
+    if (a0) {
+      V8<T>::ld(a0 + o, v);
+    }
+    if (a1) {
+      V8<T>::ld(a1 + o, q);
+#pragma unroll
+      for (int k = 0; k < VN; ++k) v[k] += q[k];
+    }
+    if (a2) {
+      V8<T>::ld(a2 + o, q);
+#pragma unroll
+      for (int k = 0; k < VN; ++k) v[k] += q[k];
+    }
+    if (part) {
+      V8<T>::ld(part + r * pitch, q);
+#pragma unroll
+      for (int k = 0; k < VN; ++k) v[k] += q[k];
+    }
+    V8<T>::st(out + o, v);
+  }
+}
+extern "C" int ge_token_grad_sum(const void* a0, const void* a1, const void* a2, const void* const* parts, const long* pitch, const long* col,
+                                 const long* level_starts, int n_parts, void* out, int B, long N, int C, int dtype, void* stream) {
+  if (!out || B <= 0 || N <= 0 || C <= 0 || n_parts < 0 || n_parts > GE_NECK_MAX_LEVELS || (!a0 && !a1 && !a2 && !n_parts)) return GE_ERR_BAD_ARG;
+  if (n_parts && (!parts || !pitch || !col)) return GE_ERR_BAD_ARG;
+  const long whole[2] = {0, N};
+  NhLevels lv;
+  NhParts pt = {};
+  long longest;
+  if (!nh_levels(n_parts ? level_starts : whole, n_parts ? n_parts : 1, N, lv, longest)) return GE_ERR_BAD_ARG;
+  if (dtype != GE_F32 && dtype != GE_BF16) return GE_ERR_UNSUPPORTED;
+  const int vn = dtype == GE_F32 ? 4 : 8;
+  bool vec = true;
+  for (int l = 0; l < n_parts; ++l) {
+    const bool empty = lv.s[l + 1] == lv.s[l];
+    if ((!parts[l] && !empty) || col[l] < 0 || col[l] + C > pitch[l]) return GE_ERR_BAD_ARG;
+    vec = vec && pitch[l] % vn == 0 && col[l] % vn == 0 && nh_aligned(parts[l]);
+    pt.p[l] = parts[l]; pt.pitch[l] = pitch[l]; pt.col[l] = col[l];
+  }
+  int lpr, rpi;
+  if (!(dtype == GE_F32 ? nh_geom<float>(C, lpr, rpi) : nh_geom<bf16_t>(C, lpr, rpi)) || !vec || !nh_aligned(a0, a1, a2, out)) return GE_ERR_UNSUPPORTED;
+  const dim3 grid(nh_grid_apply((long)B * longest, rpi), n_parts ? n_parts : 1);
+  hipStream_t s = ge_stream(stream);
+  if (dtype == GE_F32) token_grad_sum_k<float><<<grid, 256, 0, s>>>((const float*)a0, (const float*)a1, (const float*)a2, pt, n_parts > 0, (float*)out, B, N, C, lv, lpr, rpi);
+  else token_grad_sum_k<bf16_t><<<grid, 256, 0, s>>>((const bf16_t*)a0, (const bf16_t*)a1, (const bf16_t*)a2, pt, n_parts > 0, (bf16_t*)out, B, N, C, lv, lpr, rpi);
+  GE_LAUNCH_CHECK();
+  return GE_OK;
+}
+
 template <typename T> struct Gelu;
 template <> struct Gelu<float> {
   static __device__ __forceinline__ float f(float x) { return 0.5f * x * (1.f + erff(x * 0.70710678118654752f)); }
diff --git a/gedepth_amd/depth/models/necks/hahi.py b/gedepth_amd/depth/models/necks/hahi.py
--- a/gedepth_amd/depth/models/necks/hahi.py
+++ b/gedepth_amd/depth/models/necks/hahi.py
@@ -5,6 +5,7 @@
 import torch.nn.functional as F
 
 from .... import kernels as K
+from .... import neck_kernels as NK
 from ....kernels import add_rows, concat_tokens_map, ms_deform_attn_raw, residual_dropout, tokens_from_map
 from ....mmrt import bricks
 from ....mmrt.bricks import BaseModule, ConvModule, build_positional_encoding, xavier_init
@@ -123,6 +124,7 @@
         self.multi_att = MultiScaleDeformableAttention(**att)
         self.self_attn = MultiScaleDeformableAttention(**att)
         self._ref_cache = {}
+        self._pos_cache = {}
         self._order_cache = {}
 
     ORDER_REFRESH = 64
@@ -166,22 +168,53 @@
             self._ref_cache[key] = ref
         return self._ref_cache[key]
 
+    def _level_pos_rows(self, shapes, device):
+        key = (tuple(shapes), str(device))
+        if key not in self._pos_cache:
+            if len(self._pos_cache) >= 8:
+                self._pos_cache.clear()
+            self._pos_cache[key] = torch.cat([self.trans_positional_encoding.grid(h, w, device).flatten(2)[0].t() for h, w in shapes], 0).contiguous()
+        return self._pos_cache[key]
+
+    def _level_tokens(self, feats_trans):
+        if not (self.training and 'neck_levels' not in K.DISABLED and all(ft.is_cuda and K._is_cl(ft) for ft in feats_trans)
+                and self.level_embed.dtype == torch.float32 and len(feats_trans) <= min(self.level_embed.shape[0], NK.MAX_LEVELS)):
+            return None, None
+        slopes = [m._fused_bn_slope() if m.with_norm else None for m in self.trans_proj]
+        if any(s is None for s in slopes):
+            return None, None
+        pre = [m.conv_only(ft) for m, ft in zip(self.trans_proj, feats_trans)]
+        if not (NK.bn_act_levels_ok(pre) and pre[0].shape[1] % 8 == 0):
+            return None, pre
+        return NK.bn_act_levels(pre, [m.norm for m in self.trans_proj], slopes), pre
+
     def forward(self, inputs):
         assert len(inputs) == len(self.in_channels)
         feats = [conv(x) for conv, x in zip(self.lateral_convs, inputs)]
         feat_conv, feats_trans = feats[0], feats[1:]
         bs = feat_conv.shape[0]
         dev = feat_conv.device
-        shapes, srcs, poss = [], [], []
-        for i, ft in enumerate(feats_trans):
-            h, w = ft.shape[2:]
-            shapes.append((h, w))
-            pos = self.trans_positional_encoding.grid(h, w, dev).flatten(2).transpose(1, 2)
-            poss.append(pos + self.level_embed[i].view(1, 1, -1))
-            srcs.append(self.trans_proj[i](ft).flatten(2).transpose(1, 2))
-        src_flatten = torch.cat(srcs, 1)
-        pos_flatten = torch.cat(poss, 1)
-        if self.self_att:
+        shapes = [tuple(ft.shape[2:]) for ft in feats_trans]
+        level_rows = [h * w for h, w in shapes]
+        src_flatten, pre = self._level_tokens(feats_trans)
+        levels = src_flatten is not None
+        if not levels:
+            srcs, poss = [], []
+            for i, ft in enumerate(feats_trans):
+                h, w = shapes[i]
+                pos = self.trans_positional_encoding.grid(h, w, dev).flatten(2).transpose(1, 2)
+                poss.append(pos + self.level_embed[i].view(1, 1, -1))
+                srcs.append((self.trans_proj[i](ft) if pre is None else self.trans_proj[i].norm_act(pre[i])).flatten(2).transpose(1, 2))
+            src_flatten = torch.cat(srcs, 1)
+            pos_flatten = torch.cat(poss, 1)
+        if self.self_att and levels:
+            q_in, v_in, id_in = NK.fan_out(src_flatten, 3) if 'neck_fanin' not in K.DISABLED else (src_flatten,) * 3
+            ref = self._pixel_centres(shapes, dev).expand(bs, -1, -1, -1)
+            query = NK.add_rows_levels(q_in, self._level_pos_rows(shapes, dev), self.level_embed, level_rows)
+            order = (K.msda_tile_order(shapes, dev) if (os.environ.get('GE_MSDA_MM_SELF') == '1' and src_flatten.dtype == torch.bfloat16) else None)
+            src = self.self_attn(query, value=v_in, identity=id_in, query_pos=None, reference_points=ref, spatial_shapes=shapes,
+                                 query_shapes=shapes, query_order=order)
+        elif self.self_att:
             ref = self._pixel_centres(shapes, dev).expand(bs, -1, -1, -1)
             order = (K.msda_tile_order(shapes, dev) if (os.environ.get('GE_MSDA_MM_SELF') == '1' and src_flatten.is_cuda
                                                         and src_flatten.dtype == torch.bfloat16) else None)
@@ -190,6 +223,10 @@
         else:
             src = src_flatten
 
+        if levels and 'neck_fanin' not in K.DISABLED and src.dtype in (torch.float32, torch.bfloat16):
+            src_value, *pieces = NK.fan_out_levels(src, level_rows)
+        else:
+            src_value, pieces = src, torch.split(src, level_rows, dim=1)
         h, w = feat_conv.shape[2:]
         pos_map = self.conv_positional_encoding.grid(h, w, dev) if self.cross_att else None
         query = None
@@ -204,10 +241,10 @@
                 ref = torch.stack((torch.mv(pm.t(), w[0]), torch.mv(pm.t(), w[1])), -1).add(b).sigmoid()[None]
             order = self._cross_order(ref[0], shapes[0]) if (conv_skip.is_cuda and src.dtype == torch.bfloat16) else None
             ref = ref[:, :, None, :].expand(bs, -1, len(shapes), 2)
-            fused = self.multi_att.forward_map(conv_skip, pos_map, src, ref, shapes, concat_with=feat_conv, query_order=order, query=query)
+            fused = self.multi_att.forward_map(conv_skip, pos_map, src_value, ref, shapes, concat_with=feat_conv, query_order=order, query=query)
         else:
             fused = torch.cat([conv_skip, feat_conv], dim=1)
         outs = [self.conv_fusion(fused)]
-        for i, (ft, piece) in enumerate(zip(feats_trans, torch.split(src, [h * w for h, w in shapes], dim=1))):
+        for i, (ft, piece) in enumerate(zip(feats_trans, pieces)):
             outs.append(self.trans_fusion[i](concat_tokens_map(piece, ft, tokens_first=False)))
         return tuple(outs)
diff --git a/gedepth_amd/hip.py b/gedepth_amd/hip.py
--- a/gedepth_amd/hip.py
+++ b/gedepth_amd/hip.py
@@ -11,6 +11,7 @@
 EXTRA_HEADERS = {'BATCH_SIGNATURES': 'gedepth_batch.h'}
 SCENE_HEADERS = {'SCENE_SIGNATURES': 'gedepth_scene.h'}
 STRATA_HEADERS = {'STRATA_SIGNATURES': 'gedepth_strata.h'}
+NECK_HEADERS = {'NECK_SIGNATURES': 'gedepth_neck.h'}
 GE_F32, GE_BF16 = 0, 1
 GE_COLORIZE_VMIN_DATA, GE_COLORIZE_VMAX_DATA, GE_COLORIZE_EQUAL = 1, 2, 4
 
@@ -39,7 +40,7 @@
     return sigs
 
 
-for _table, _header in {**HEADERS, **EXTRA_HEADERS, **SCENE_HEADERS, **STRATA_HEADERS}.items():
+for _table, _header in {**HEADERS, **EXTRA_HEADERS, **SCENE_HEADERS, **STRATA_HEADERS, **NECK_HEADERS}.items():
     with open(os.path.join(os.path.dirname(_HERE), 'include', _header)) as _fh:
         globals()[_table] = parse_header(_fh.read())
 
@@ -58,7 +59,7 @@
                 f'{LIB_PATH} is missing: the gfx950 HIP kernels are not built. '
                 f'Run gedepth_amd/csrc/build.sh (hipcc --offload-arch=gfx950). There is no CPU/eager fallback.')
         handle = ctypes.CDLL(LIB_PATH)
-        for table in (*HEADERS, *EXTRA_HEADERS, *SCENE_HEADERS, *STRATA_HEADERS):
+        for table in (*HEADERS, *EXTRA_HEADERS, *SCENE_HEADERS, *STRATA_HEADERS, *NECK_HEADERS):
             for name, (res, args) in globals()[table].items():
                 fn = getattr(handle, name)
                 fn.restype, fn.argtypes = res, args
diff --git a/gedepth_amd/mmrt/bricks.py b/gedepth_amd/mmrt/bricks.py
--- a/gedepth_amd/mmrt/bricks.py
+++ b/gedepth_amd/mmrt/bricks.py
@@ -397,18 +397,21 @@
             return float(self.activate.negative_slope)
         return None
 
+    def conv_only(self, x):
+        if x.is_cuda and self.conv.bias is None:
+            from .. import kernels
+            if kernels.conv3x3_ok(self.conv, x):
+                return kernels.conv3x3(self.conv, x)
+            return kernels.conv_lib(self.conv, x)
+        return self.conv(x)
+
     def forward(self, x):
         slope = self._fused_slope() if x.is_cuda else None
         if slope is not None:
             return conv_bias_act(self.conv, x, slope)
-        if x.is_cuda and self.conv.bias is None:
-            from .. import kernels
-            if kernels.conv3x3_ok(self.conv, x):
-                x = kernels.conv3x3(self.conv, x)
-            else:
-                x = kernels.conv_lib(self.conv, x)
-        else:
-            x = self.conv(x)
+        return self.norm_act(self.conv_only(x))
+
+    def norm_act(self, x):
         if x.is_cuda and self.with_norm and x.dtype in (torch.float32, torch.bfloat16):
             slope = self._fused_bn_slope()
             if slope is not None:
diff --git a/gedepth_amd/neck_kernels.py b/gedepth_amd/neck_kernels.py
--- /dev/null
+++ b/gedepth_amd/neck_kernels.py
@@ -0,0 +1,216 @@
+import ctypes
+
+import torch
+
+from . import hip
+from .kernels import _c, _cl_ok, _es, _f32, _launch, _tag
+
+MAX_LEVELS = 8
+_WS = {}
+
+
+def _starts(level_rows, n_levels=None):
+    n_levels = len(level_rows) if n_levels is None else n_levels
+    if not 1 <= len(level_rows) <= n_levels <= MAX_LEVELS or any(r < 0 for r in level_rows):
+        raise ValueError(f'a level table takes 1 .. {MAX_LEVELS} levels of non-negative size, got {tuple(level_rows)} for {n_levels} levels')
+    starts, acc = [0], 0
+    for l in range(n_levels):
+        acc += int(level_rows[l]) if l < len(level_rows) else 0
+        starts.append(acc)
+    return (ctypes.c_long * len(starts))(*starts), n_levels, acc
+
+
+def _workspace(device, C, K):
+    key = (device, hip.stream(), C, K)
+    ws = _WS.get(key)
+    if ws is None:
+        ws = _WS[key] = torch.empty(int(hip.lib().ge_nhwc_workspace(C, K)), device=device, dtype=torch.uint8)
+    return ws
+
+
+def _vec_ok(t):
+    vn = 8 if t.dtype == torch.bfloat16 else 4
+    return t.is_cuda and t.dtype in (_f32, torch.bfloat16) and t.shape[-1] % vn == 0 and t.shape[-1] // vn <= 256
+
+
+class _BNActLevels(torch.autograd.Function):
+
+    @staticmethod
+    def forward(ctx, meta, *tensors):
+        L = len(meta)
+        xs, wb = tensors[:L], tensors[L:]
+        B, C = xs[0].shape[:2]
+        rows = [x.shape[2] * x.shape[3] for x in xs]
+        N, es, dt = sum(rows), _es(xs[0]), hip.dtype_code(xs[0])
+        out = torch.empty(B, N, C, device=xs[0].device, dtype=xs[0].dtype)
+        stats = torch.empty(L, 2, C, device=out.device, dtype=_f32)
+        ws = torch.empty(int(hip.lib().ge_nhwc_workspace(C, 2)), device=out.device, dtype=torch.uint8)
+        saved, start = [], 0
+        for l, (x, n) in enumerate(zip(xs, rows)):
+            assert _cl_ok(x) and tuple(x.shape[:2]) == (B, C) and x.dtype == out.dtype
+            w, b = _c(wb[2 * l].detach().to(_f32)), _c(wb[2 * l + 1].detach().to(_f32))
+            rm, rv, eps, momentum, slope = meta[l]
+            _launch(f'bn_act_rows_fwd[{B}x{C}x{x.shape[2]}x{x.shape[3]} {_tag(x)}]', 3 * x.numel() * es, 'ge_bn_act_nhwc_fwd_rows', x.data_ptr(),
+                    hip.ptr(w), hip.ptr(b), out.data_ptr() + start * C * es, n, N, hip.ptr(stats[l, 0]), hip.ptr(stats[l, 1]), hip.ptr(rm, _f32),
+                    hip.ptr(rv, _f32), hip.ptr(ws), B * n, C, eps, momentum, slope, dt, hip.stream())
+            saved += [x, w, b]
+            start += n
+        ctx.save_for_backward(stats, *saved)
+        ctx.slopes = [m[4] for m in meta]
+        return out
+
+    @staticmethod
+    def backward(ctx, d):
+        stats, saved = ctx.saved_tensors[0], ctx.saved_tensors[1:]
+        L = len(ctx.slopes)
+        x0 = saved[0]
+        B, C = x0.shape[:2]
+        d = _c(d.to(x0.dtype))
+        N, es, dt = d.shape[1], _es(x0), hip.dtype_code(x0)
+        dwb = torch.empty(L, 2, C, device=d.device, dtype=_f32)
+        ws = torch.empty(int(hip.lib().ge_nhwc_workspace(C, 2)), device=d.device, dtype=torch.uint8)
+        dxs, start = [], 0
+        for l in range(L):
+            x, w, b = saved[3 * l:3 * l + 3]
+            n = x.shape[2] * x.shape[3]
+            dx = torch.empty_like(x)
+            _launch(f'bn_act_rows_bwd[{B}x{C}x{x.shape[2]}x{x.shape[3]} {_tag(x)}]', 5 * x.numel() * es, 'ge_bn_act_nhwc_bwd_rows',
+                    d.data_ptr() + start * C * es, n, N, x.data_ptr(), hip.ptr(w), hip.ptr(b), hip.ptr(stats[l, 0]), hip.ptr(stats[l, 1]),
+                    dx.data_ptr(), hip.ptr(dwb[l, 0]), hip.ptr(dwb[l, 1]), hip.ptr(ws), B * n, C, ctx.slopes[l], dt, hip.stream())
+            dxs.append(dx)
+            start += n
+        return (None, *dxs, *(dwb[l, k] for l in range(L) for k in range(2)))
+
+
+def bn_act_levels_ok(maps):
+    x0 = maps[0]
+    return (1 <= len(maps) <= MAX_LEVELS and all(_cl_ok(x) and x.dtype == x0.dtype and tuple(x.shape[:2]) == tuple(x0.shape[:2]) for x in maps))
+
+
+def bn_act_levels(maps, bns, slopes):
+    meta = [(bn.running_mean, bn.running_var, float(bn.eps), float(bn.momentum), float(s)) for bn, s in zip(bns, slopes)]
+    out = _BNActLevels.apply(meta, *maps, *(p for bn in bns for p in (bn.weight, bn.bias)))
+    for bn in bns:
+        bn.num_batches_tracked.add_(1)
+    return out
+
+
+def level_colsum(x, level_rows, n_levels=None):
+    B, N, C = x.shape
+    starts, L, total = _starts(level_rows, n_levels)
+    assert total == N and x.is_contiguous()
+    out = torch.empty(L, C, device=x.device, dtype=_f32)
+    _launch(f'level_colsum[{B}x{N}x{C} {_tag(x)}]', x.numel() * _es(x), 'ge_level_colsum', hip.ptr(x, name='x'), B, N, C,
+            ctypes.cast(starts, ctypes.c_void_p), L, hip.ptr(out), hip.ptr(_workspace(x.device, C, L)), hip.dtype_code(x), hip.stream())
+    return out
+
+
+class _AddRowsLevels(torch.autograd.Function):
+
+    @staticmethod
+    def forward(ctx, tok, pos_rows, emb, level_rows):
+        tok = _c(tok)
+        B, N, C = tok.shape
+        starts, L, total = _starts(level_rows, emb.shape[0])
+        assert total == N and tuple(pos_rows.shape) == (N, C) and emb.shape[1] == C
+        out = torch.empty_like(tok)
+        _launch(f'add_rows_levels[{B}x{N}x{C} {_tag(tok)}]', 2 * tok.numel() * _es(tok) + N * C * 4, 'ge_add_rows_levels', hip.ptr(tok, name='tokens'),
+                hip.ptr(pos_rows, _f32, 'pos'), hip.ptr(_c(emb.detach()), _f32, 'emb'), hip.ptr(out), B, N, C, ctypes.cast(starts, ctypes.c_void_p), L,
+                hip.dtype_code(tok), hip.stream())
+        ctx.level_rows, ctx.n_levels = tuple(level_rows), L
+        return out
+
+    @staticmethod
+    def backward(ctx, d):
+        d_emb = level_colsum(_c(d), ctx.level_rows, ctx.n_levels) if ctx.needs_input_grad[2] else None
+        return d, None, d_emb, None
+
+
+def add_rows_levels(tokens, pos_rows, emb, level_rows):
+    return _AddRowsLevels.apply(tokens, pos_rows, emb, tuple(int(r) for r in level_rows))
+
+
+def _part_args(part, B, C):
+    if isinstance(part, tuple):
+        wide, col = part
+        assert wide.dim() == 2 and wide.is_contiguous() and wide.shape[0] % B == 0 and 0 <= col and col + C <= wide.shape[1]
+        return wide.shape[0] // B, wide.data_ptr(), wide.shape[1], int(col), wide.dtype
+    assert part.shape[0] == B and part.shape[2] == C
+    n, pitch = part.shape[1], part.stride(1)
+    if part.stride(2) != 1 or pitch < C or (B > 1 and part.stride(0) != n * pitch):
+        return None
+    return n, part.data_ptr(), pitch, 0, part.dtype
+
+
+def token_grad_sum(addends, parts=None):
+    addends = [_c(a) for a in addends]
+    ref = addends[0] if addends else parts[0]
+    B, C = ref.shape[0], ref.shape[2]
+    assert len(addends) <= 3 and _vec_ok(ref) and all(a.shape == ref.shape and a.dtype == ref.dtype for a in addends)
+    es, vn = _es(ref), 16 // _es(ref)
+    n_parts, ptrs, pitch, col, starts, keep = 0, None, None, None, None, []
+    if parts:
+        args = []
+        for p in parts:
+            a = _part_args(p, B, C)
+            if a is None or a[1] % 16 or a[2] % vn or a[3] % vn:
+                p = p.contiguous()
+                keep.append(p)
+                a = (p.shape[1], p.data_ptr(), C, 0, p.dtype)
+            assert a[4] == ref.dtype
+            args.append(a)
+        starts, n_parts, N = _starts([a[0] for a in args])
+        ptrs = (ctypes.c_void_p * n_parts)(*(a[1] for a in args))
+        pitch = (ctypes.c_long * n_parts)(*(a[2] for a in args))
+        col = (ctypes.c_long * n_parts)(*(a[3] for a in args))
+    else:
+        N = ref.shape[1]
+    assert not addends or ref.shape[1] == N
+    out = torch.empty(B, N, C, device=ref.device, dtype=ref.dtype)
+    a = [hip.ptr(t, name='addend') for t in addends] + [None] * (3 - len(addends))
+    cast = lambda arr: None if arr is None else ctypes.cast(arr, ctypes.c_void_p)
+    _launch(f'token_grad_sum[{B}x{N}x{C} {_tag(ref)} {len(addends)}{"+parts" if parts else ""}]', (len(addends) + bool(parts) + 1) * out.numel() * es,
+            'ge_token_grad_sum', a[0], a[1], a[2], cast(ptrs), cast(pitch), cast(col), cast(starts), n_parts, hip.ptr(out), B, N, C,
+            hip.dtype_code(ref), hip.stream())
+    return out
+
+
+class _FanOut(torch.autograd.Function):
+
+    @staticmethod
+    def forward(ctx, x, n):
+        ctx.set_materialize_grads(False)
+        return tuple(x.view_as(x) for _ in range(n))
+
+    @staticmethod
+    def backward(ctx, *gs):
+        gs = [g for g in gs if g is not None]
+        if not gs:
+            return None, None
+        return (gs[0] if len(gs) == 1 else token_grad_sum(gs)), None
+
+
+def fan_out(x, n):
+    assert 1 <= n <= 3
+    return _FanOut.apply(x, n)
+
+
+class _FanOutLevels(torch.autograd.Function):
+
+    @staticmethod
+    def forward(ctx, x, level_rows):
+        ctx.set_materialize_grads(False)
+        ctx.meta = (tuple(x.shape), x.dtype, x.device, level_rows)
+        return (x.view_as(x), *x.split(list(level_rows), 1))
+
+    @staticmethod
+    def backward(ctx, g, *parts):
+        (B, N, C), dtype, device, level_rows = ctx.meta
+        if all(p is None for p in parts):
+            return g, None
+        parts = [torch.zeros(B, n, C, device=device, dtype=dtype) if p is None else p for p, n in zip(parts, level_rows)]
+        return token_grad_sum([] if g is None else [g], parts), None
+
+
+def fan_out_levels(x, level_rows):
+    return _FanOutLevels.apply(x, tuple(int(r) for r in level_rows))
diff --git a/include/gedepth_neck.h b/include/gedepth_neck.h
--- /dev/null
+++ b/include/gedepth_neck.h
@@ -0,0 +1,32 @@
+#ifndef GEDEPTH_NECK_H
+#define GEDEPTH_NECK_H
+
+#include <stddef.h>
+#include <stdint.h>
+
+#ifdef __cplusplus
+extern "C" {
+#endif
+
+#define GE_NECK_MAX_LEVELS 8
+
+int ge_bn_act_nhwc_fwd_rows(const void* x, const float* gamma, const float* beta, void* y, long rows_per_image, long image_stride,
+                            float* save_mean, float* save_rstd, float* running_mean, float* running_var, void* workspace, long rows, int C,
+                            float eps, float momentum, float slope, int dtype, void* stream);
+int ge_bn_act_nhwc_bwd_rows(const void* dy, long rows_per_image, long image_stride, const void* x, const float* gamma, const float* beta,
+                            const float* save_mean, const float* save_rstd, void* dx, float* dgamma, float* dbeta, void* workspace, long rows,
+                            int C, float slope, int dtype, void* stream);
+
+int ge_add_rows_levels(const void* x, const float* pos, const float* emb, void* out, int B, long N, int C, const long* level_starts,
+                       int n_levels, int dtype, void* stream);
+
+int ge_level_colsum(const void* x, int B, long N, int C, const long* level_starts, int n_levels, float* out, void* workspace, int dtype,
+                    void* stream);
+
+int ge_token_grad_sum(const void* a0, const void* a1, const void* a2, const void* const* parts, const long* pitch, const long* col,
+                      const long* level_starts, int n_parts, void* out, int B, long N, int C, int dtype, void* stream);
+
+#ifdef __cplusplus
+}
+#endif
+#endif
```

Measured after the change: 175.0 img/s, median of 6. 2.1% higher.
